# HJakeCunningham/ASVGP

Hardware: NVIDIA B200
Metric: elbo_grad_datapoints_per_s (higher is better)
Workload: dtype f64

## Files before the change

asvgp_b200/csrc/band_engine.cuh:

```cuda
#pragma once
#include "common.cuh"
#include "dual.cuh"

namespace asvgp {

struct ChunkLayout {
    int M, K, P;
    int base, rem;
    ASVGP_HD int size(int p) const { return base + (p < rem ? 1 : 0); }
    ASVGP_HD int start(int p) const { return p * (base + K) + (p < rem ? p : rem); }
    ASVGP_HD int sep_start(int q) const { return start(q) + size(q); }
    ASVGP_HD int max_size() const { return base + (rem > 0 ? 1 : 0); }
    ASVGP_HD int n_reduced() const { return (P - 1) * K; }
};

inline ChunkLayout make_layout(int M, int K, int P) {
    ChunkLayout L;
    L.M = M; L.K = K;
    while (P > 1 && (M - (P - 1) * K) / P < K + 1) --P;
    L.P = P;
    const int interior = M - (P - 1) * K;
    L.base = interior / P;
    L.rem = interior % P;
    return L;
}

inline int default_chunks(int M, int K) {
    if (M < 16 * (K + 1)) return 1;
    int P = M / (4 * (K + 1));
    if (P > 128) P = 128;
    if (P < 1) P = 1;
    return P;
}

template <class T, int K, bool SPIKE = true>
struct ColumnStore {
    T* rec;
    int n_steps, P;
    static constexpr int kFields = SPIKE ? 2 * K + 2 : K + 2;
    static constexpr int kY = kFields - 1;
    ASVGP_HD T& at(int field, int j, int p) const { return rec[((size_t)field * n_steps + j) * P + p]; }
    ASVGP_HD static size_t count(int n_steps, int P) { return (size_t)kFields * n_steps * P; }
};

template <class T, int K>
struct ChunkSchur {
    T logdet, quad;
    T Dend[K][K];
    T rend[K];
    T E[K][K];
    T SLL[K][K];
    T rhsL[K];
    int info;
};

template <class T, int K>
struct WindowRow {
    T a[K + 1];
    T r;
};

template <class T, int K, class MatFn, class RhsFn>
ASVGP_HD void fetch_row(MatFn& A, RhsFn& rhs, int g, WindowRow<T, K>& row) {
#pragma unroll
    for (int b = 0; b <= K; ++b) row.a[b] = A(K - b, g + 1 + b);
    row.r = rhs(g + 1 + K);
}

template <class T, int K, bool SPIKE, bool STORE, class MatFn, class RhsFn, class Store>
ASVGP_HD void eliminate_columns(int g0, int n, int n_steps, MatFn A, RhsFn rhs, const Store& store,
                                int p, ChunkSchur<T, K>& out) {
    T W[K + 1][K + 1];
    T r[K + 1];
    T c[SPIKE ? K : 1][K + 1];
#pragma unroll
    for (int a = 0; a <= K; ++a) {
#pragma unroll
        for (int b = 0; b <= a; ++b) W[a][b] = A(a - b, g0 + b);
        r[a] = rhs(g0 + a);
    }
    if (SPIKE) {
#pragma unroll
        for (int rho = 0; rho < K; ++rho)
#pragma unroll
            for (int a = 0; a <= K; ++a)
                c[rho][a] = (a <= rho) ? A(a + K - rho, g0 - K + rho) : zero_of<T>();
    }
    LogAccum<T> logdet;
    logdet.init();
    T quad = zero_of<T>();
    T SLL[K][K], rhsL[K];
#pragma unroll
    for (int a = 0; a < K; ++a) {
        rhsL[a] = zero_of<T>();
#pragma unroll
        for (int b = 0; b < K; ++b) SLL[a][b] = zero_of<T>();
    }
    int info = 0;

    WindowRow<T, K> rowA, rowB;
    fetch_row<T, K>(A, rhs, g0, rowA);
    fetch_row<T, K>(A, rhs, g0 + 1, rowB);

    auto step = [&](int j, const WindowRow<T, K>& row) {
        const int g = g0 + j;
        if (!(value_of(W[0][0]) > 0.0) && info == 0) info = g + 1;
        const T ip = rsqrt_of(W[0][0]);
        logdet.add(W[0][0], ip);
        T l[K + 1];
#pragma unroll
        for (int a = 1; a <= K; ++a) l[a] = W[a][0] * ip;
        const T yj = r[0] * ip;
        quad += yj * yj;
        T X[SPIKE ? K : 1];
        if (SPIKE) {
#pragma unroll
            for (int rho = 0; rho < K; ++rho) {
                X[rho] = c[rho][0] * ip;
                rhsL[rho] += X[rho] * yj;
#pragma unroll
                for (int r2 = 0; r2 <= rho; ++r2) SLL[rho][r2] += X[rho] * X[r2];
            }
        }
        if (STORE) {
            store.at(0, j, p) = ip;
#pragma unroll
            for (int a = 1; a <= K; ++a) store.at(a, j, p) = l[a];
            if (SPIKE) {
#pragma unroll
                for (int rho = 0; rho < K; ++rho) store.at(K + 1 + rho, j, p) = X[rho];
            }
            store.at(Store::kY, j, p) = yj;
        }
#pragma unroll
        for (int a = 1; a <= K; ++a) {
#pragma unroll
            for (int b = 1; b <= a; ++b) W[a - 1][b - 1] = W[a][b] - l[a] * l[b];
            r[a - 1] = r[a] - l[a] * yj;
            if (SPIKE) {
#pragma unroll
                for (int rho = 0; rho < K; ++rho) c[rho][a - 1] = c[rho][a] - l[a] * X[rho];
            }
        }
#pragma unroll
        for (int b = 0; b <= K; ++b) W[K][b] = row.a[b];
        r[K] = row.r;
        if (SPIKE) {
#pragma unroll
            for (int rho = 0; rho < K; ++rho) c[rho][K] = zero_of<T>();
        }
    };

    for (int j = 0; j < n_steps; j += 2) {
        WindowRow<T, K> nextA, nextB;
        fetch_row<T, K>(A, rhs, g0 + j + 2, nextA);
        if (j < n) step(j, rowA);
        fetch_row<T, K>(A, rhs, g0 + j + 3, nextB);
        if (j + 1 < n) step(j + 1, rowB);
        rowA = nextA;
        rowB = nextB;
    }
    out.logdet = logdet.result();
    out.quad = quad;
    out.info = info;
#pragma unroll
    for (int a = 0; a < K; ++a) {
        out.rend[a] = r[a];
        out.rhsL[a] = rhsL[a];
#pragma unroll
        for (int b = 0; b < K; ++b) {
            out.Dend[a][b] = (b <= a) ? W[a][b] : zero_of<T>();
            out.SLL[a][b] = SLL[a][b];
            out.E[a][b] = SPIKE ? c[b][a] : zero_of<T>();
        }
    }
}

template <class T, int K, class Store>
ASVGP_HD void backsolve_serial(int n, const Store& store, T* x) {
    T xw[K + 1];
#pragma unroll
    for (int a = 0; a <= K; ++a) xw[a] = zero_of<T>();
    for (int j = n - 1; j >= 0; --j) {
        T acc = store.at(Store::kY, j, 0);
#pragma unroll
        for (int a = 1; a <= K; ++a) acc -= store.at(a, j, 0) * xw[a];
        const T xj = acc * store.at(0, j, 0);
#pragma unroll
        for (int a = K; a >= 2; --a) xw[a] = xw[a - 1];
        xw[1] = xj;
        x[j] = xj;
    }
}

template <class T>
struct BandSink {
    T* sig; int M;
    ASVGP_HD void operator()(int d, int col, const T& v) const { sig[(size_t)d * M + col] = v; }
};

template <class T, int K, class Store, class Sink>
ASVGP_HD void selinv_serial(int n, const Store& store, Sink& sink) {
    T Z[K][K];
#pragma unroll
    for (int a = 0; a < K; ++a)
#pragma unroll
        for (int b = 0; b < K; ++b) Z[a][b] = zero_of<T>();
    for (int j = n - 1; j >= 0; --j) {
        const T ip = store.at(0, j, 0);
        T l[K], w[K];
#pragma unroll
        for (int a = 0; a < K; ++a) l[a] = store.at(a + 1, j, 0);
        T dot = zero_of<T>();
#pragma unroll
        for (int a = 0; a < K; ++a) {
            T acc = zero_of<T>();
#pragma unroll
            for (int b = 0; b < K; ++b) acc += Z[a][b] * l[b];
            w[a] = acc;
            dot += l[a] * acc;
        }
        const T ip2 = ip * ip;
        const T sjj = ip2 + dot * ip2;
        sink(0, j, sjj);
        T col[K];
#pragma unroll
        for (int a = 0; a < K; ++a) {
            col[a] = -(w[a] * ip);
            if (j + 1 + a < n) sink(a + 1, j, col[a]);
        }
#pragma unroll
        for (int a = K - 1; a >= 1; --a)
#pragma unroll
            for (int b = K - 1; b >= 1; --b) Z[a][b] = Z[a - 1][b - 1];
        Z[0][0] = sjj;
#pragma unroll
        for (int a = 1; a < K; ++a) { Z[a][0] = col[a - 1]; Z[0][a] = col[a - 1]; }
    }
}

template <class T, int K, bool SOLVE, bool SELINV, class Sink>
ASVGP_HD void chunk_backward(const ChunkLayout& lay, int p, int n_steps, const ColumnStore<T, K, true>& store,
                             const T* x_red, const T* sig_red, T* x_out, Sink& sink) {
    constexpr int KR = 2 * K - 1;
    const int n = lay.size(p), s = lay.start(p), M = lay.M, nred = lay.n_reduced();
    const bool has_left = p > 0, has_right = p < lay.P - 1;
    (void)KR;
    T xw[K + 1], xL[K];
    T Z[2 * K][2 * K];
#pragma unroll
    for (int a = 0; a < K; ++a) {
        xw[a + 1] = (SOLVE && has_right) ? x_red[p * K + a] : zero_of<T>();
        xL[a] = (SOLVE && has_left) ? x_red[(p - 1) * K + a] : zero_of<T>();
    }
    xw[0] = zero_of<T>();
    if (SELINV) {
#pragma unroll
        for (int a = 0; a < 2 * K; ++a)
#pragma unroll
            for (int b = 0; b < 2 * K; ++b) Z[a][b] = zero_of<T>();
#pragma unroll
        for (int a = 0; a < K; ++a) {
#pragma unroll
            for (int b = 0; b <= a; ++b) {
                if (has_right) { Z[a][b] = sig_red[(size_t)(a - b) * nred + p * K + b]; Z[b][a] = Z[a][b]; }
                if (has_left) {
                    Z[K + a][K + b] = sig_red[(size_t)(a - b) * nred + (p - 1) * K + b];
                    Z[K + b][K + a] = Z[K + a][K + b];
                }
            }
#pragma unroll
            for (int rho = 0; rho < K; ++rho) {
                if (has_left && has_right) {
                    Z[a][K + rho] = sig_red[(size_t)(K + a - rho) * nred + (p - 1) * K + rho];
                    Z[K + rho][a] = Z[a][K + rho];
                }
            }
        }
    }
    struct Rec { T ip; T lv[2 * K]; T y; };
    auto fetch = [&](int j, Rec& rec) {
        const int jj = j < 0 ? 0 : (j >= n_steps ? n_steps - 1 : j);
        rec.ip = store.at(0, jj, p);
#pragma unroll
        for (int a = 0; a < K; ++a) {
            rec.lv[a] = store.at(a + 1, jj, p);
            rec.lv[K + a] = store.at(K + 1 + a, jj, p);
        }
        rec.y = store.at(ColumnStore<T, K, true>::kY, jj, p);
    };
    auto step = [&](int j, const Rec& rec) {
        const int g = s + j;
        const T ip = rec.ip;
        if (SOLVE) {
            T acc = rec.y;
#pragma unroll
            for (int a = 0; a < K; ++a) { acc -= rec.lv[a] * xw[a + 1]; acc -= rec.lv[K + a] * xL[a]; }
            const T xj = acc * ip;
#pragma unroll
            for (int a = K; a >= 2; --a) xw[a] = xw[a - 1];
            xw[1] = xj;
            x_out[g] = xj;
        }
        if (SELINV) {
            T w[2 * K];
            T dot = zero_of<T>();
#pragma unroll
            for (int a = 0; a < 2 * K; ++a) {
                T acc = zero_of<T>();
#pragma unroll
                for (int b = 0; b < 2 * K; ++b) acc += Z[a][b] * rec.lv[b];
                w[a] = acc;
                dot += rec.lv[a] * acc;
            }
            const T ip2 = ip * ip;
            const T sjj = ip2 + dot * ip2;
            sink(0, g, sjj);
            T col[2 * K];
#pragma unroll
            for (int a = 0; a < 2 * K; ++a) col[a] = -(w[a] * ip);
#pragma unroll
            for (int a = 0; a < K; ++a) {
                if (g + 1 + a < M) sink(a + 1, g, col[a]);
                if (has_left && j <= a) sink(j + K - a, s - K + a, col[K + a]);
            }
#pragma unroll
            for (int a = K - 1; a >= 1; --a) {
#pragma unroll
                for (int b = K - 1; b >= 1; --b) Z[a][b] = Z[a - 1][b - 1];
#pragma unroll
                for (int rho = 0; rho < K; ++rho) { Z[a][K + rho] = Z[a - 1][K + rho]; Z[K + rho][a] = Z[a][K + rho]; }
            }
            Z[0][0] = sjj;
#pragma unroll
            for (int a = 1; a < K; ++a) { Z[a][0] = col[a - 1]; Z[0][a] = col[a - 1]; }
#pragma unroll
            for (int rho = 0; rho < K; ++rho) { Z[0][K + rho] = col[K + rho]; Z[K + rho][0] = col[K + rho]; }
        }
    };
    Rec recA, recB;
    const int top = ((n_steps + 1) & ~1) - 1;
    fetch(top, recA);
    fetch(top - 1, recB);
    for (int j = top; j >= 0; j -= 2) {
        Rec nextA, nextB;
        fetch(j - 2, nextA);
        if (j < n) step(j, recA);
        fetch(j - 3, nextB);
        if (j - 1 < n && j - 1 >= 0) step(j - 1, recB);
        recA = nextA;
        recB = nextB;
    }
}

}

namespace asvgp {

template <class T, int B>
struct CrNode {
    T D[B][B];
    T E[B][B];
    T Wa[B][B];
    T Wb[B][B];
    T Sa[B][B];
    T Sb[B][B];
    T r[B];
    T ip[B];
    T logdet, quad;
    int info;
};

#if defined(__CUDACC__)
template <class P> __device__ __forceinline__ P* cluster_peer(P* p, int rank) {
    unsigned long long out;
    asm volatile("mapa.u64 %0, %1, %2;" : "=l"(out) : "l"((unsigned long long)p), "r"(rank));
    return reinterpret_cast<P*>(out);
}
#endif

template <class T, int K>
struct ChainWork {
    ColumnStore<T, K, true> cols;
    ChunkSchur<T, K>* schur;
    CrNode<T, K>* nodes;
    T* x_red;
    T* sig_red;
    int per_cta = 0;
    ASVGP_HD ChunkSchur<T, K>& sch(int p) const {
#if defined(__CUDA_ARCH__)
        if (per_cta > 0) return *cluster_peer(schur + p % per_cta, p / per_cta);
#endif
        return schur[p];
    }
    ASVGP_HD CrNode<T, K>& node(int i) const {
#if defined(__CUDA_ARCH__)
        if (per_cta > 0) return *cluster_peer(nodes + i % per_cta, i / per_cta);
#endif
        return nodes[i];
    }
};

template <class T, int K>
struct ChainSmall {
    ASVGP_HD static size_t align16(size_t n) { return (n + 15) & ~(size_t)15; }
    ASVGP_HD static size_t head_bytes(int P) {
        const size_t nred = (size_t)(P - 1) * K + 1;
        const size_t a = align16((size_t)P * sizeof(ChunkSchur<T, K>));
        const size_t b = align16((size_t)(2 * K) * nred * sizeof(T)) + align16(nred * sizeof(T));
        return a > b ? a : b;
    }
    ASVGP_HD static size_t bytes(int P) { return head_bytes(P) + align16((size_t)(P > 1 ? P - 1 : 1) * sizeof(CrNode<T, K>)); }
    ASVGP_HD static void carve(int P, char* base, ChainWork<T, K>& w) {
        const size_t nred = (size_t)(P - 1) * K + 1;
        w.schur = reinterpret_cast<ChunkSchur<T, K>*>(base);
        w.sig_red = reinterpret_cast<T*>(base);
        w.x_red = reinterpret_cast<T*>(base + align16((size_t)(2 * K) * nred * sizeof(T)));
        w.nodes = reinterpret_cast<CrNode<T, K>*>(base + head_bytes(P));
    }
};

template <class T, int K>
struct ChainTotals { T logdet, quad; int info; };

template <class T, int K, bool STORE, class MatFn, class RhsFn>
ASVGP_HD void chain_phase1(const ChunkLayout& lay, int p, MatFn A, RhsFn rhs, const ChainWork<T, K>& w) {
    const int n_steps = lay.max_size();
    if (lay.P == 1) eliminate_columns<T, K, false, STORE>(0, lay.M, n_steps, A, rhs, w.cols, 0, w.sch(0));
    else eliminate_columns<T, K, true, STORE>(lay.start(p), lay.size(p), n_steps, A, rhs, w.cols, p, w.sch(p));
}

template <class T, int K>
ASVGP_HD void cr_assemble(const ChunkLayout& lay, int q, const ChainWork<T, K>& w) {
    const ChunkSchur<T, K>& left = w.sch(q);
    const ChunkSchur<T, K>& right = w.sch(q + 1);
    CrNode<T, K>& nd = w.node(q);
#pragma unroll
    for (int a = 0; a < K; ++a) {
        nd.r[a] = left.rend[a] - right.rhsL[a];
#pragma unroll
        for (int b = 0; b < K; ++b) {
            nd.D[a][b] = (b <= a) ? left.Dend[a][b] - right.SLL[a][b] : zero_of<T>();
            nd.E[a][b] = left.E[a][b];
        }
    }
    nd.logdet = zero_of<T>();
    nd.quad = zero_of<T>();
    nd.info = 0;
}

template <class T, int K>
ASVGP_HD void cr_eliminate(int n, int s, int i, int g_offset, const ChainWork<T, K>& w) {
    CrNode<T, K>& nd = w.node(i);
    const bool has_a = s > 0 && i - s >= 0, has_b = s > 0 && i + s < n;
    T D[K][K], r[K], ipv[K], E[K][K], Eb[K][K];
#pragma unroll
    for (int a = 0; a < K; ++a) {
        r[a] = nd.r[a];
#pragma unroll
        for (int b = 0; b < K; ++b) {
            D[a][b] = (b <= a) ? nd.D[a][b] : zero_of<T>();
            E[a][b] = has_a ? nd.E[a][b] : zero_of<T>();
            Eb[a][b] = has_b ? w.node(i + s).E[a][b] : zero_of<T>();
        }
    }
    LogAccum<T> logdet;
    logdet.init();
    T quad = zero_of<T>();
    int info = 0;
#pragma unroll
    for (int j = 0; j < K; ++j) {
        T d = D[j][j];
#pragma unroll
        for (int q = 0; q < j; ++q) d -= D[j][q] * D[j][q];
        if (!(value_of(d) > 0.0) && info == 0) info = g_offset + i * K + j + 1;
        const T ip = rsqrt_of(d);
        logdet.add(d, ip);
        ipv[j] = ip;
        D[j][j] = d * ip;
#pragma unroll
        for (int rr = j + 1; rr < K; ++rr) {
            T v = D[rr][j];
#pragma unroll
            for (int q = 0; q < j; ++q) v -= D[rr][q] * D[j][q];
            D[rr][j] = v * ip;
        }
        T y = r[j];
#pragma unroll
        for (int q = 0; q < j; ++q) y -= D[j][q] * r[q];
        y = y * ip;
        r[j] = y;
        quad += y * y;
    }
    T Wa[K][K], Wb[K][K];
#pragma unroll
    for (int x = 0; x < K; ++x)
#pragma unroll
        for (int j = 0; j < K; ++j) {
            T va = E[j][x], vb = Eb[x][j];
#pragma unroll
            for (int q = 0; q < j; ++q) { va -= D[j][q] * Wa[x][q]; vb -= D[j][q] * Wb[x][q]; }
            Wa[x][j] = va * ipv[j];
            Wb[x][j] = vb * ipv[j];
        }
#pragma unroll
    for (int a = 0; a < K; ++a) {
        nd.r[a] = r[a];
        nd.ip[a] = ipv[a];
#pragma unroll
        for (int b = 0; b < K; ++b) {
            if (b <= a) nd.D[a][b] = D[a][b];
            if (has_a) nd.Wa[a][b] = Wa[a][b];
            if (has_b) nd.Wb[a][b] = Wb[a][b];
        }
    }
    nd.logdet = logdet.result();
    nd.quad = quad;
    if (info != 0 && nd.info == 0) nd.info = info;
}

template <class T, int K>
ASVGP_HD void cr_update(int n, int s, int c, const ChainWork<T, K>& w) {
    CrNode<T, K>& nd = w.node(c);
    const bool has_p = c + s < n, has_m = c - s >= 0, has_a = c - 2 * s >= 0;
    T D[K][K], r[K], Wp[K][K], yp[K], Wm[K][K], Wma[K][K], ym[K];
#pragma unroll
    for (int a = 0; a < K; ++a) {
        r[a] = nd.r[a];
        yp[a] = has_p ? w.node(c + s).r[a] : zero_of<T>();
        ym[a] = has_m ? w.node(c - s).r[a] : zero_of<T>();
#pragma unroll
        for (int b = 0; b < K; ++b) {
            D[a][b] = (b <= a) ? nd.D[a][b] : zero_of<T>();
            Wp[a][b] = has_p ? w.node(c + s).Wa[a][b] : zero_of<T>();
            Wm[a][b] = has_m ? w.node(c - s).Wb[a][b] : zero_of<T>();
            Wma[a][b] = (has_m && has_a) ? w.node(c - s).Wa[a][b] : zero_of<T>();
        }
    }
#pragma unroll
    for (int x = 0; x < K; ++x) {
        T rr = r[x];
#pragma unroll
        for (int j = 0; j < K; ++j) { rr -= Wp[x][j] * yp[j]; rr -= Wm[x][j] * ym[j]; }
        nd.r[x] = rr;
#pragma unroll
        for (int y = 0; y <= x; ++y) {
            T v = D[x][y];
#pragma unroll
            for (int j = 0; j < K; ++j) { v -= Wp[x][j] * Wp[y][j]; v -= Wm[x][j] * Wm[y][j]; }
            nd.D[x][y] = v;
        }
        if (has_m) {
#pragma unroll
            for (int y = 0; y < K; ++y) {
                T v = zero_of<T>();
#pragma unroll
                for (int j = 0; j < K; ++j) v -= Wm[x][j] * Wma[y][j];
                nd.E[x][y] = v;
            }
        }
    }
}

template <class T, int K, bool SOLVE, bool SELINV>
ASVGP_HD void cr_back(int n, int s, int i, const ChainWork<T, K>& w) {
    CrNode<T, K>& nd = w.node(i);
    const bool has_a = s > 0 && i - s >= 0, has_b = s > 0 && i + s < n;
    const CrNode<T, K>& na = w.node(has_a ? i - s : i);
    const CrNode<T, K>& nb = w.node(has_b ? i + s : i);
    T L[K][K], ipv[K], Wa[K][K], Wb[K][K];
#pragma unroll
    for (int a = 0; a < K; ++a) {
        ipv[a] = nd.ip[a];
#pragma unroll
        for (int b = 0; b < K; ++b) {
            L[a][b] = (b <= a) ? nd.D[a][b] : zero_of<T>();
            Wa[a][b] = has_a ? nd.Wa[a][b] : zero_of<T>();
            Wb[a][b] = has_b ? nd.Wb[a][b] : zero_of<T>();
        }
    }
    if (SOLVE) {
        T t[K], xa[K], xb[K];
#pragma unroll
        for (int j = 0; j < K; ++j) {
            t[j] = nd.r[j];
            xa[j] = has_a ? na.r[j] : zero_of<T>();
            xb[j] = has_b ? nb.r[j] : zero_of<T>();
        }
#pragma unroll
        for (int j = 0; j < K; ++j) {
            T v = t[j];
#pragma unroll
            for (int x = 0; x < K; ++x) { v -= Wa[x][j] * xa[x]; v -= Wb[x][j] * xb[x]; }
            t[j] = v;
        }
#pragma unroll
        for (int j = K - 1; j >= 0; --j) {
            T v = t[j];
#pragma unroll
            for (int q = j + 1; q < K; ++q) v -= L[q][j] * t[q];
            t[j] = v * ipv[j];
        }
#pragma unroll
        for (int j = 0; j < K; ++j) nd.r[j] = t[j];
    }
    if (SELINV) {
        const bool both = has_a && has_b;
        const bool a_is_odd = both && (((i - s) / (2 * s)) & 1);
        T Saa[K][K], Sbb[K][K], Sba[K][K];
#pragma unroll
        for (int x = 0; x < K; ++x)
#pragma unroll
            for (int y = 0; y < K; ++y) {
                Saa[x][y] = has_a ? na.D[x][y] : zero_of<T>();
                Sbb[x][y] = has_b ? nb.D[x][y] : zero_of<T>();
                Sba[x][y] = both ? (a_is_odd ? na.Sb[x][y] : nb.Sa[y][x]) : zero_of<T>();
            }
        T Li[K][K];
#pragma unroll
        for (int c = 0; c < K; ++c)
#pragma unroll
            for (int r = 0; r < K; ++r) {
                if (r < c) { Li[r][c] = zero_of<T>(); continue; }
                T v = (r == c) ? make_scalar<T>(1.0, 0.0) : zero_of<T>();
#pragma unroll
                for (int q = c; q < r; ++q) v -= L[r][q] * Li[q][c];
                Li[r][c] = v * ipv[r];
            }
        T Ya[K][K], Yb[K][K];
#pragma unroll
        for (int x = 0; x < K; ++x)
#pragma unroll
            for (int c = 0; c < K; ++c) {
                T va = zero_of<T>(), vb = zero_of<T>();
#pragma unroll
                for (int j = c; j < K; ++j) { va += Wa[x][j] * Li[j][c]; vb += Wb[x][j] * Li[j][c]; }
                Ya[x][c] = va;
                Yb[x][c] = vb;
            }
        T Sai[K][K], Sbi[K][K];
#pragma unroll
        for (int x = 0; x < K; ++x)
#pragma unroll
            for (int c = 0; c < K; ++c) {
                T va = zero_of<T>(), vb = zero_of<T>();
#pragma unroll
                for (int y = 0; y < K; ++y) {
                    va -= Saa[x][y] * Ya[y][c];
                    va -= Sba[y][x] * Yb[y][c];
                    vb -= Sba[x][y] * Ya[y][c];
                    vb -= Sbb[x][y] * Yb[y][c];
                }
                Sai[x][c] = va;
                Sbi[x][c] = vb;
            }
#pragma unroll
        for (int c = 0; c < K; ++c)
#pragma unroll
            for (int c2 = 0; c2 < K; ++c2) {
                T v = zero_of<T>();
#pragma unroll
                for (int r = 0; r < K; ++r) {
                    if (r >= c && r >= c2) v += Li[r][c] * Li[r][c2];
                }
#pragma unroll
                for (int x = 0; x < K; ++x) { v -= Ya[x][c] * Sai[x][c2]; v -= Yb[x][c] * Sbi[x][c2]; }
                nd.D[c][c2] = v;
                if (has_a) nd.Sa[c][c2] = Sai[c][c2];
                if (has_b) nd.Sb[c][c2] = Sbi[c][c2];
            }
    }
}

template <class T, int K, bool SOLVE, bool SELINV>
ASVGP_HD void cr_export(const ChunkLayout& lay, int q, const ChainWork<T, K>& w) {
    const int nred = lay.n_reduced();
    const CrNode<T, K>& nd = w.node(q);
    if (SOLVE) {
#pragma unroll
        for (int a = 0; a < K; ++a) w.x_red[q * K + a] = nd.r[a];
    }
    if (SELINV) {
#pragma unroll
        for (int a = 0; a < K; ++a)
#pragma unroll
            for (int b = 0; b <= a; ++b) w.sig_red[(size_t)(a - b) * nred + q * K + b] = nd.D[a][b];
        if (q >= 1) {
            const bool q_odd = q & 1;
            const CrNode<T, K>& prev = w.node(q - 1);
#pragma unroll
            for (int a = 0; a < K; ++a)
#pragma unroll
                for (int rho = 0; rho < K; ++rho)
                    w.sig_red[(size_t)(K + a - rho) * nred + (q - 1) * K + rho] = q_odd ? nd.Sa[rho][a] : prev.Sb[a][rho];
        }
    }
}

template <class T, int K>
ASVGP_HD ChainTotals<T, K> chain_totals(const ChunkLayout& lay, const ChainWork<T, K>& w) {
    ChainTotals<T, K> tot;
    tot.logdet = zero_of<T>();
    tot.quad = zero_of<T>();
    tot.info = 0;
    for (int p = 0; p < lay.P; ++p) {
        tot.logdet += w.sch(p).logdet;
        tot.quad += w.sch(p).quad;
        if (w.sch(p).info != 0 && (tot.info == 0 || w.sch(p).info < tot.info)) tot.info = w.sch(p).info;
    }
    for (int q = 0; q + 1 < lay.P; ++q) {
        tot.logdet += w.node(q).logdet;
        tot.quad += w.node(q).quad;
        if (w.node(q).info != 0 && tot.info == 0) tot.info = w.node(q).info;
    }
    return tot;
}

ASVGP_HD int cr_top_stride(int n) {
    int s = 1;
    while (2 * s < n) s *= 2;
    return n > 1 ? s : 0;
}

template <class T, int K, bool SOLVE, bool SELINV, class Sink>
ASVGP_HD void chain_phase3(const ChunkLayout& lay, int p, const ChainWork<T, K>& w, T* x_out, Sink& sink) {
    const int n_steps = lay.max_size();
    if (lay.P == 1) {
        if (SOLVE) backsolve_serial<T, K>(lay.M, w.cols, x_out);
        if (SELINV) selinv_serial<T, K>(lay.M, w.cols, sink);
        return;
    }
    const int nred = lay.n_reduced();
    if (p < lay.P - 1) {
        const int g = lay.sep_start(p);
        for (int a = 0; a < K; ++a) {
            if (SOLVE) x_out[g + a] = w.x_red[p * K + a];
            if (SELINV)
                for (int b = 0; b <= a; ++b)
                    sink(a - b, g + b, w.sig_red[(size_t)(a - b) * nred + p * K + b]);
        }
    }
    chunk_backward<T, K, SOLVE, SELINV>(lay, p, n_steps, w.cols, w.x_red, w.sig_red, x_out, sink);
}

}
```

asvgp_b200/csrc/banded_1d.cu:

```cuda
#include <cooperative_groups.h>
#include <cuda_runtime.h>

#include <cstdio>
#include <cstdlib>

#include <algorithm>

#include "band_engine.cuh"
#include "../../include/asvgp_b200.h"

namespace asvgp {

constexpr int kChainThreads = 128;

__device__ __forceinline__ void pdl_wait() { asm volatile("griddepcontrol.wait;" ::: "memory"); }
__device__ __forceinline__ void pdl_launch_dependents() { asm volatile("griddepcontrol.launch_dependents;" ::: "memory"); }
constexpr int kMaxTerms = 12;

struct KuuTerms {
    int n_terms;
    double coef[kMaxTerms];
    double dcoef[kMaxTerms];
};

__global__ void __launch_bounds__(256) kuu_assemble_kernel(const double* __restrict__ tables, KuuTerms terms,
                                                           int64_t band_elems, double* __restrict__ Kuu,
                                                           double* __restrict__ dKuu) {
    for (int64_t i = blockIdx.x * (int64_t)blockDim.x + threadIdx.x; i < band_elems;
         i += (int64_t)gridDim.x * blockDim.x) {
        double v = 0.0, dv = 0.0;
        for (int t = 0; t < terms.n_terms; ++t) {
            const double s = __ldg(tables + (int64_t)t * band_elems + i);
            v = __dadd_rn(v, __dmul_rn(terms.coef[t], s));
            dv = __dadd_rn(dv, __dmul_rn(terms.dcoef[t], s));
        }
        Kuu[i] = v;
        if (dKuu != nullptr) dKuu[i] = dv;
    }
}

template <class T> struct BandMat;
template <> struct BandMat<Dual<1>> {
    const double* Kuu; const double* dKuu; const double* G;
    double beta, tb; int use_dK; int M;
    __device__ __forceinline__ Dual<1> operator()(int d, int j) const {
        const bool ok = (j >= 0) & (j + d < M);
        const size_t i = ok ? (size_t)d * M + j : 0;
        const double kv = __ldg(Kuu + i);
        const double dk = use_dK ? __ldg(dKuu + i) : 0.0;
        const double g = (G != nullptr) ? __ldg(G + i) : 0.0;
        Dual<1> r;
        r.v = ok ? fma(beta, g, kv) : 0.0;
        r.d[0] = ok ? fma(tb, g, dk) : 0.0;
        return r;
    }
};
template <> struct BandMat<double> {
    const double* Kuu; const double* dKuu; const double* G;
    double beta, tb; int use_dK; int M;
    __device__ __forceinline__ double operator()(int d, int j) const {
        const bool ok = (j >= 0) & (j + d < M);
        const size_t i = ok ? (size_t)d * M + j : 0;
        const double kv = __ldg(Kuu + i);
        const double g = (G != nullptr) ? __ldg(G + i) : 0.0;
        return ok ? fma(beta, g, kv) : 0.0;
    }
};
template <class T> struct VecRhs {
    const double* b; int M; int use;
    __device__ __forceinline__ T operator()(int j) const {
        const bool ok = (use != 0) & (j >= 0) & (j < M);
        const double v = __ldg(b + (ok ? j : 0));
        return make_scalar<T>(ok ? v : 0.0, 0.0);
    }
};

template <class T, int K>
struct RowsMat {
    const T* rows; int g0, P, p, n_rho;
    __device__ __forceinline__ T operator()(int d, int col) const {
        const int rho = col + d - g0;
        const bool ok = (rho >= 0) & (rho < n_rho);
        const T v = rows[ok ? ((size_t)rho * (K + 1) + (K - d)) * P + p : (size_t)p];
        return ok ? v : zero_of<T>();
    }
};
template <class T>
struct RowsRhs {
    const T* r; int g0, P, p, n_rho;
    __device__ __forceinline__ T operator()(int j) const {
        const int rho = j - g0;
        const bool ok = (rho >= 0) & (rho < n_rho);
        const T v = r[ok ? (size_t)rho * P + p : (size_t)p];
        return ok ? v : zero_of<T>();
    }
};
__host__ __device__ inline int chain_n_rho(const ChunkLayout& lay, int K) { return lay.max_size() + K + 4; }
template <class T, int K>
__host__ __device__ inline size_t chain_rows_count(const ChunkLayout& lay) {
    return (size_t)chain_n_rho(lay, K) * (K + 2) * lay.P;
}

template <class T> struct ChainSpec { BandMat<T> A; VecRhs<T> rhs; };

constexpr int kTraceBlocks = 64, kTraceThreads = 256, kTraceUnroll = 4;
struct TraceJob {
    const double* kstate;
    const double* G;
    double* tr_part;
    int M, K, first_block;
};
__device__ __forceinline__ void trace_partial(const double* __restrict__ kstate, const double* __restrict__ G, int M, int K, int block,
                                              double* __restrict__ tr_part) {
    __shared__ double s_tr[2][kTraceThreads / 32];
    const Dual<1>* kinv = reinterpret_cast<const Dual<1>*>(kstate + 16);
    double tr = 0.0, dtr_dl = 0.0;
    const int band = (K + 1) * M, stride = kTraceThreads * kTraceBlocks;
    for (int i0 = block * kTraceThreads + threadIdx.x; i0 < band; i0 += stride * kTraceUnroll) {
        Dual<1> sv[kTraceUnroll];
        double gv[kTraceUnroll];
#pragma unroll
        for (int u = 0; u < kTraceUnroll; ++u) {
            const int i = i0 + u * stride;
            const int d = i / M, col = i - d * M;
            const bool ok = i < band && col + d < M;
            sv[u] = kinv[ok ? i : 0];
            gv[u] = ok ? (d == 0 ? 1.0 : 2.0) * G[i] : 0.0;
        }
#pragma unroll
        for (int u = 0; u < kTraceUnroll; ++u) {
            if (gv[u] != 0.0) { tr = fma(sv[u].v, gv[u], tr); dtr_dl = fma(sv[u].d[0], gv[u], dtr_dl); }
        }
    }
#pragma unroll
    for (int o = 16; o > 0; o >>= 1) {
        tr += __shfl_xor_sync(0xffffffffu, tr, o);
        dtr_dl += __shfl_xor_sync(0xffffffffu, dtr_dl, o);
    }
    if ((threadIdx.x & 31) == 0) { s_tr[0][threadIdx.x >> 5] = tr; s_tr[1][threadIdx.x >> 5] = dtr_dl; }
    __syncthreads();
    if (threadIdx.x == 0) {
        tr = 0.0; dtr_dl = 0.0;
        for (int i = 0; i < kTraceThreads / 32; ++i) { tr += s_tr[0][i]; dtr_dl += s_tr[1][i]; }
        tr_part[2 * block] = tr; tr_part[2 * block + 1] = dtr_dl;
    }
}

template <class T, int K, int NCHAINS>
__global__ void __launch_bounds__(256) chain_rows_kernel(ChunkLayout lay, ChainSpec<T> s0, ChainSpec<T> s1, ChainSpec<T> s2, ChainSpec<T> s3,
                                                         T* __restrict__ out, unsigned* __restrict__ zero_me = nullptr,
                                                         TraceJob trace = TraceJob{nullptr, nullptr, nullptr, 0, 0, 0}) {
    pdl_launch_dependents();
    if (zero_me != nullptr && blockIdx.x == 0 && threadIdx.x == 0) *zero_me = 0u;
    if (trace.kstate != nullptr && (int)blockIdx.x >= trace.first_block) {
        trace_partial(trace.kstate, trace.G, trace.M, trace.K, (int)blockIdx.x - trace.first_block, trace.tr_part);
        return;
    }
    const unsigned n_rho = chain_n_rho(lay, K), P = lay.P;
    const unsigned per_chain = (unsigned)chain_rows_count<T, K>(lay);
    const unsigned total = per_chain * NCHAINS;
    const unsigned n_row_blocks = trace.kstate != nullptr ? (unsigned)trace.first_block : gridDim.x;
    for (unsigned t = blockIdx.x * blockDim.x + threadIdx.x; t < total; t += n_row_blocks * blockDim.x) {
        const unsigned chain = t / per_chain;
        const unsigned e = t - chain * per_chain;
        const ChainSpec<T>& sp = chain == 0 ? s0 : (chain == 1 ? s1 : (chain == 2 ? s2 : s3));
        const unsigned q = e / P;
        const int p = (int)(e - q * P);
        const int g0 = P > 1 ? lay.start(p) : 0;
        if (q < n_rho * (K + 1)) {
            const int rho = (int)(q / (K + 1)), bidx = (int)(q - (unsigned)rho * (K + 1));
            const int row = g0 + rho, col = row - K + bidx;
            out[t] = sp.A(K - bidx, col);
        } else {
            const int rho = (int)(q - n_rho * (K + 1));
            out[t] = sp.rhs(g0 + rho);
        }
    }
}

template <class T, int K>
struct ChainPlan {
    static size_t bytes(const ChunkLayout& lay) {
        const size_t n = ColumnStore<T, K, true>::count(lay.max_size(), lay.P) * sizeof(T);
        return (n + 255) & ~(size_t)255;
    }
    static ColumnStore<T, K, true> carve(const ChunkLayout& lay, char* base) {
        return ColumnStore<T, K, true>{reinterpret_cast<T*>(base), lay.max_size(), lay.P};
    }
};

constexpr size_t kChainSmemLimit = 200 * 1024;

template <class T, int K, bool STORE, bool SOLVE, bool SELINV, class Mat, class Rhs, class Sink>
__device__ __forceinline__ void run_chain(const ChunkLayout& lay, const ColumnStore<T, K, true>& cols, char* smem,
                                          Mat A, Rhs rhs, T* x_out, Sink& sink, ChainTotals<T, K>* tot,
                                          long long* clk) {
    const int p = threadIdx.x;
    ChainWork<T, K> w;
    w.cols = cols;
    ChainSmall<T, K>::carve(lay.P, smem, w);
    if (p == 0 && clk) clk[0] = clock64();
    if (p < lay.P) chain_phase1<T, K, STORE>(lay, p, A, rhs, w);
    __syncthreads();
    if (p == 0 && clk) clk[1] = clock64();
    const int n = lay.P - 1;
    if (p < n) cr_assemble<T, K>(lay, p, w);
    __syncthreads();
    for (int s = 1; s < n; s *= 2) {
        if (p < n && (p & (2 * s - 1)) == s) cr_eliminate<T, K>(n, s, p, lay.M, w);
        __syncthreads();
        if (p < n && (p & (2 * s - 1)) == 0) cr_update<T, K>(n, s, p, w);
        __syncthreads();
    }
    if (p == 0) {
        if (n > 0) cr_eliminate<T, K>(n, 0, 0, lay.M, w);
        *tot = chain_totals<T, K>(lay, w);
        if ((SOLVE || SELINV) && n > 0) cr_back<T, K, SOLVE, SELINV>(n, 0, 0, w);
    }
    __syncthreads();
    if ((SOLVE || SELINV) && n > 0) {
        for (int s = cr_top_stride(n); s >= 1; s /= 2) {
            if (p < n && (p & (2 * s - 1)) == s) cr_back<T, K, SOLVE, SELINV>(n, s, p, w);
            __syncthreads();
        }
        if (p < n) cr_export<T, K, SOLVE, SELINV>(lay, p, w);
        __syncthreads();
    }
    if (p == 0 && clk) clk[2] = clock64();
    if ((SOLVE || SELINV) && p < lay.P) chain_phase3<T, K, SOLVE, SELINV>(lay, p, w, x_out, sink);
    __syncthreads();
    if (p == 0 && clk) clk[3] = clock64();
}

template <class T, int K, bool STORE, bool SOLVE, bool SELINV, class MakeMat, class MakeRhs, class MakeSink>
__device__ __forceinline__ void run_chain_cluster(const ChunkLayout& lay, const ColumnStore<T, K, true>& cols, char* smem, T* red_scratch,
                                                  MakeMat make_A, MakeRhs make_rhs, MakeSink make_sink, T* x_out,
                                                  ChainTotals<T, K>* tot, long long* clk) {
    namespace cg = cooperative_groups;
    cg::cluster_group cluster = cg::this_cluster();
    const int rank = (int)cluster.block_rank(), n_cta = (int)cluster.num_blocks();
    const int tid = threadIdx.x;
    const int per = kChainThreads;
    const int p = rank * per + tid;
    ChainWork<T, K> w;
    w.cols = cols;
    ChainSmall<T, K>::carve(per + 1, smem, w);
    w.per_cta = per;
    const size_t nred = (size_t)lay.n_reduced();
    w.sig_red = red_scratch;
    w.x_red = red_scratch + (size_t)(2 * K) * nred;
#ifdef ASVGP_CHAIN_TRACE
    __shared__ long long s_trace[64];
    int n_trace = 0;
#define ASVGP_STAMP() do { if (rank == 0 && tid == 0 && n_trace < 64) s_trace[n_trace++] = clock64(); } while (0)
#else
#define ASVGP_STAMP() do {} while (0)
#endif
    cluster.sync();
    ASVGP_STAMP();
    if (rank == 0 && tid == 0 && clk) clk[0] = clock64();
    if (p < lay.P) chain_phase1<T, K, STORE>(lay, p, make_A(p), make_rhs(p), w);
    cluster.sync();
    ASVGP_STAMP();
    if (rank == 0 && tid == 0 && clk) clk[1] = clock64();
    const int n = lay.P - 1;
    if (p < n) cr_assemble<T, K>(lay, p, w);
    cluster.sync();
    ASVGP_STAMP();
    for (int s = 1; s < n; s *= 2) {
        if (p < n && (p & (2 * s - 1)) == s) cr_eliminate<T, K>(n, s, p, lay.M, w);
        cluster.sync();
        ASVGP_STAMP();
        if (p < n && (p & (2 * s - 1)) == 0) cr_update<T, K>(n, s, p, w);
        cluster.sync();
        ASVGP_STAMP();
    }
    if (p == 0 && n > 0) cr_eliminate<T, K>(n, 0, 0, lay.M, w);
    cluster.sync();
    ASVGP_STAMP();
    {
        T ld = zero_of<T>(), qd = zero_of<T>();
        int info = 0;
        if (p < lay.P) { const ChunkSchur<T, K>& c = w.sch(p); ld += c.logdet; qd += c.quad; info = c.info; }
        if (p < n) { const CrNode<T, K>& nd = w.node(p); ld += nd.logdet; qd += nd.quad; if (info == 0) info = nd.info; }
        double v[4] = {value_of(ld), tangent_of(ld, 0), value_of(qd), tangent_of(qd, 0)};
        unsigned uinfo = info == 0 ? 0xffffffffu : (unsigned)info;
#pragma unroll
        for (int o = 16; o > 0; o >>= 1) {
#pragma unroll
            for (int i = 0; i < 4; ++i) v[i] += __shfl_xor_sync(0xffffffffu, v[i], o);
            uinfo = min(uinfo, __shfl_xor_sync(0xffffffffu, uinfo, o));
        }
        __shared__ double s_tot[kChainThreads / 32][4];
        __shared__ unsigned s_info[kChainThreads / 32];
        __shared__ double s_cta[5];
        if ((tid & 31) == 0) { for (int i = 0; i < 4; ++i) s_tot[tid >> 5][i] = v[i]; s_info[tid >> 5] = uinfo; }
        __syncthreads();
        if (tid == 0) {
            double a[4] = {0, 0, 0, 0};
            unsigned ui = 0xffffffffu;
            for (int wv = 0; wv < kChainThreads / 32; ++wv) { for (int i = 0; i < 4; ++i) a[i] += s_tot[wv][i]; ui = min(ui, s_info[wv]); }
            for (int i = 0; i < 4; ++i) s_cta[i] = a[i];
            s_cta[4] = (double)ui;
        }
        cluster.sync();
        ASVGP_STAMP();
        if (rank == 0 && tid == 0) {
            double a[4] = {0, 0, 0, 0};
            double ui = 4294967295.0;
            for (int r = 0; r < n_cta; ++r) {
                const double* q = cluster_peer(s_cta, r);
                for (int i = 0; i < 4; ++i) a[i] += q[i];
                ui = q[4] < ui ? q[4] : ui;
            }
            tot->logdet = make_scalar<T>(a[0], a[1]);
            tot->quad = make_scalar<T>(a[2], a[3]);
            tot->info = ui >= 4294967295.0 ? 0 : (int)ui;
        }
    }
    if ((SOLVE || SELINV) && n > 0) {
        if (p == 0) cr_back<T, K, SOLVE, SELINV>(n, 0, 0, w);
        cluster.sync();
        ASVGP_STAMP();
        for (int s = cr_top_stride(n); s >= 1; s /= 2) {
            if (p < n && (p & (2 * s - 1)) == s) cr_back<T, K, SOLVE, SELINV>(n, s, p, w);
            cluster.sync();
            ASVGP_STAMP();
        }
        if (p < n) cr_export<T, K, SOLVE, SELINV>(lay, p, w);
        __threadfence();
        cluster.sync();
        ASVGP_STAMP();
    }
    if (rank == 0 && tid == 0 && clk) clk[2] = clock64();
    if ((SOLVE || SELINV) && p < lay.P) {
        auto sink = make_sink(p);
        chain_phase3<T, K, SOLVE, SELINV>(lay, p, w, x_out, sink);
    }
    cluster.sync();
    ASVGP_STAMP();
    if (rank == 0 && tid == 0 && clk) clk[3] = clock64();
#ifdef ASVGP_CHAIN_TRACE
    if (rank == 0 && tid == 0) {
        for (int i = 1; i < n_trace; ++i) printf("trace blk=%d SELINV=%d P=%d step=%d %lld\n", (int)blockIdx.x, (int)SELINV, lay.P, i, s_trace[i] - s_trace[i - 1]);
    }
#endif
#undef ASVGP_STAMP
}

template <int K>
struct ElboArgs {
    ChunkLayout lay;
    int first_chain;
    ColumnStore<Dual<1>, K, true> cols[2];
    double* partial[2];
    const Dual<1>* rows;
    Dual<1>* kinv;
};

template <int K>
__global__ void __launch_bounds__(kChainThreads) elbo_chains_kernel(ElboArgs<K> a) {
    using T = Dual<1>;
    extern __shared__ __align__(16) char smem[];
    const int slot = blockIdx.x, chain = a.first_chain + slot, p = threadIdx.x;
    const ChunkLayout lay = a.lay;
    const int M = lay.M;
    __shared__ ChainTotals<T, K> tot;
    __shared__ long long clk[4];
    double* out = a.partial[slot];
    pdl_launch_dependents();
    pdl_wait();

    const int n_rho = chain_n_rho(lay, K), g0 = lay.P > 1 ? lay.start(p < lay.P ? p : 0) : 0, pp = p < lay.P ? p : 0;
    const T* tab = a.rows + (size_t)slot * chain_rows_count<T, K>(lay);
    const RowsMat<T, K> A{tab, g0, lay.P, pp, n_rho};
    const RowsRhs<T> rhs{tab + (size_t)n_rho * (K + 1) * lay.P, g0, lay.P, pp, n_rho};
    if (chain == 0) {
        BandSink<T> sink{a.kinv, M};
        run_chain<T, K, true, false, true>(lay, a.cols[slot], smem, A, rhs, static_cast<T*>(nullptr), sink, &tot, clk);
    } else {
        BandSink<T> no_sink{nullptr, M};
        run_chain<T, K, false, false, false>(lay, a.cols[slot], smem, A, rhs, static_cast<T*>(nullptr), no_sink, &tot, clk);
    }
    if (p == 0) {
        out[0] = tot.logdet.v; out[1] = tot.logdet.d[0];
        out[2] = tot.quad.v;   out[3] = tot.quad.d[0];
        out[6] = (double)tot.info;
        const long long t_end = clock64();
        out[8] = (double)(clk[1] - clk[0]); out[9] = (double)(clk[2] - clk[1]);
        out[10] = (double)(clk[3] - clk[2]); out[11] = (double)(t_end - clk[3]);
    }
}

template <int K, int NCTA>
__global__ void __cluster_dims__(NCTA, 1, 1) __launch_bounds__(kChainThreads) elbo_chains_cluster_kernel(ElboArgs<K> a, Dual<1>* red_scratch) {
    using T = Dual<1>;
    extern __shared__ __align__(16) char smem[];
    const int slot = blockIdx.x / NCTA, chain = a.first_chain + slot, rank = blockIdx.x % NCTA, tid = threadIdx.x;
    const ChunkLayout lay = a.lay;
    __shared__ ChainTotals<T, K> tot;
    __shared__ long long clk[4];
    double* out = a.partial[slot];
    pdl_launch_dependents();
    pdl_wait();
    const int n_rho = chain_n_rho(lay, K);
    const T* tab = a.rows + (size_t)slot * chain_rows_count<T, K>(lay);
    T* scratch = red_scratch + (size_t)slot * ((size_t)(2 * K + 1) * lay.n_reduced() + 8);
    auto g0_of = [&](int lane) { return lay.P > 1 ? lay.start(lane) : 0; };
    auto make_A = [&](int lane) { return RowsMat<T, K>{tab, g0_of(lane), lay.P, lane, n_rho}; };
    auto make_rhs = [&](int lane) { return RowsRhs<T>{tab + (size_t)n_rho * (K + 1) * lay.P, g0_of(lane), lay.P, lane, n_rho}; };
    if (chain == 0) {
        auto make_sink = [&](int) { return BandSink<T>{a.kinv, lay.M}; };
        run_chain_cluster<T, K, true, false, true>(lay, a.cols[slot], smem, scratch, make_A, make_rhs, make_sink, static_cast<T*>(nullptr), &tot, clk);
    } else {
        auto make_sink = [&](int) { return BandSink<T>{nullptr, lay.M}; };
        run_chain_cluster<T, K, false, false, false>(lay, a.cols[slot], smem, scratch, make_A, make_rhs, make_sink, static_cast<T*>(nullptr), &tot, clk);
    }
    if (rank == 0 && tid == 0) {
        out[0] = tot.logdet.v; out[1] = tot.logdet.d[0];
        out[2] = tot.quad.v;   out[3] = tot.quad.d[0];
        out[6] = (double)tot.info;
        const long long t_end = clock64();
        out[8] = (double)(clk[1] - clk[0]); out[9] = (double)(clk[2] - clk[1]);
        out[10] = (double)(clk[3] - clk[2]); out[11] = (double)(t_end - clk[3]);
    }
}

__global__ void __launch_bounds__(kTraceThreads) elbo_finalize_kernel(const double* __restrict__ kstate, double* __restrict__ partial,
                                                                      const double* __restrict__ G, const double* __restrict__ scal,
                                                                      int M, int K, double variance, double sigma2, int trace_done,
                                                                      double* __restrict__ out) {
    double* tr_part = partial + 64;
    unsigned* counter = reinterpret_cast<unsigned*>(partial + 32);
    pdl_wait();
    if (!trace_done) {
        trace_partial(kstate, G, M, K, (int)blockIdx.x, tr_part);
        if (threadIdx.x != 0) return;
        __threadfence();
        if (atomicAdd(counter, 1u) != gridDim.x - 1) return;
        __threadfence();
    } else if (threadIdx.x != 0) {
        return;
    }
    double tr = 0.0, dtr_dl = 0.0;
    for (int i = 0; i < kTraceBlocks; ++i) { tr += __ldcg(tr_part + 2 * i); dtr_dl += __ldcg(tr_part + 2 * i + 1); }
    const double* cK = kstate;
    const double* cL = partial;
    const double* cS = partial + 16;
    const double yy = scal[0], N = scal[1];
    const double v = variance, s2 = sigma2;
    const double logdetK = cK[0], dlogdetK_dl = cK[1];
    const double logdetP = cL[0], dlogdetP_dl = cL[1], Q = cL[2], dQ_dl = cL[3];
    const double dlogdetP_ds = cS[1], dQ_ds = cS[3];
    const double two_pi = 6.283185307179586476925286766559;
    const double elbo = -0.5 * N * log(two_pi * s2) - 0.5 * logdetP + 0.5 * logdetK - 0.5 * yy / s2
                        + 0.5 * Q / (s2 * s2) - 0.5 * N * v / s2 + 0.5 * tr / s2;
    const double d_l = -0.5 * dlogdetP_dl + 0.5 * dlogdetK_dl + 0.5 * dQ_dl / (s2 * s2) + 0.5 * dtr_dl / s2;
    const double d_s = -0.5 * N / s2 - 0.5 * dlogdetP_ds + 0.5 * yy / (s2 * s2) + 0.5 * dQ_ds / (s2 * s2)
                       - Q / (s2 * s2 * s2) + 0.5 * N * v / (s2 * s2) - 0.5 * tr / (s2 * s2);
    const double dlogdetP_dv = -(double)M / v - (s2 / v) * dlogdetP_ds;
    const double dQ_dv = Q / v - (s2 / v) * dQ_ds;
    const double d_v = -0.5 * dlogdetP_dv - 0.5 * (double)M / v + 0.5 * dQ_dv / (s2 * s2) - 0.5 * N / s2
                       + 0.5 * tr / (v * s2);
    out[0] = elbo; out[1] = d_v; out[2] = d_l; out[3] = d_s;
    out[4] = logdetK; out[5] = logdetP; out[6] = Q; out[7] = tr;
    double info = cK[6];
    if (info == 0.0) info = cL[6];
    if (info == 0.0) info = cS[6];
    out[8] = info;
    out[9] = cK[8]; out[10] = cK[9]; out[11] = cK[10]; out[12] = cK[11];
    out[13] = cL[8]; out[14] = cL[9];
    out[15] = dtr_dl;
}

template <int K>
struct PosteriorArgs {
    ChunkLayout lay;
    ColumnStore<double, K, true> cols[2];
    const double* Kuu; const double* G; const double* b;
    double sigma2;
    double* sigK; double* sigP; double* x;
    double* info;
    const double* rows;
};

template <int K>
__global__ void __launch_bounds__(kChainThreads) posterior_chains_kernel(PosteriorArgs<K> a) {
    using T = double;
    extern __shared__ __align__(16) char smem[];
    const int chain = blockIdx.x, p = threadIdx.x;
    const ChunkLayout lay = a.lay;
    const int M = lay.M;
    __shared__ ChainTotals<T, K> tot;
    (void)M;
    const int n_rho = chain_n_rho(lay, K), g0 = lay.P > 1 ? lay.start(p < lay.P ? p : 0) : 0, pp = p < lay.P ? p : 0;
    const T* tab = a.rows + (size_t)chain * chain_rows_count<T, K>(lay);
    const RowsMat<T, K> A{tab, g0, lay.P, pp, n_rho};
    const RowsRhs<T> rhs{tab + (size_t)n_rho * (K + 1) * lay.P, g0, lay.P, pp, n_rho};
    BandSink<T> sinkK{a.sigK, lay.M}, sinkP{a.sigP, lay.M};
    if (chain == 0) run_chain<T, K, true, false, true>(lay, a.cols[0], smem, A, rhs, static_cast<T*>(nullptr), sinkK, &tot, nullptr);
    else run_chain<T, K, true, true, true>(lay, a.cols[1], smem, A, rhs, a.x, sinkP, &tot, nullptr);
    if (p == 0) a.info[chain] = (double)tot.info;
}

__global__ void __launch_bounds__(256) posterior_combine_kernel(const double* __restrict__ sigK,
                                                                const double* __restrict__ sigP,
                                                                const double* __restrict__ x, double inv_s2, int M,
                                                                int band_elems, double* __restrict__ alpha,
                                                                double* __restrict__ S) {
    for (int i = blockIdx.x * blockDim.x + threadIdx.x; i < band_elems; i += gridDim.x * blockDim.x) {
        S[i] = sigP[i] - sigK[i];
        if (i < M) alpha[i] = x[i] * inv_s2;
    }
}


template <int K>
struct BandInvArgs {
    ChunkLayout lay;
    ColumnStore<Dual<1>, K, true> cols;
    const double* A; const double* dA;
    Dual<1>* sig;
    double* sig_val; double* sig_tan;
    double* scal;
    const Dual<1>* rows;
};

template <int K>
__global__ void __launch_bounds__(kChainThreads) band_inverse_kernel(BandInvArgs<K> a) {
    using T = Dual<1>;
    extern __shared__ __align__(16) char smem[];
    const int p = threadIdx.x;
    const ChunkLayout lay = a.lay;
    const int M = lay.M;
    __shared__ ChainTotals<T, K> tot;
    const int n_rho = chain_n_rho(lay, K), g0 = lay.P > 1 ? lay.start(p < lay.P ? p : 0) : 0, pp = p < lay.P ? p : 0;
    const RowsMat<T, K> A{a.rows, g0, lay.P, pp, n_rho};
    const RowsRhs<T> rhs{a.rows + (size_t)n_rho * (K + 1) * lay.P, g0, lay.P, pp, n_rho};
    BandSink<T> sink{a.sig, lay.M};
    run_chain<T, K, true, false, true>(lay, a.cols, smem, A, rhs, static_cast<T*>(nullptr), sink, &tot, nullptr);
    for (int i = p; i < (K + 1) * M; i += kChainThreads) {
        const T s = a.sig[i];
        a.sig_val[i] = s.v;
        a.sig_tan[i] = s.d[0];
    }
    if (p == 0) {
        a.scal[0] = tot.logdet.v; a.scal[1] = tot.logdet.d[0]; a.scal[2] = (double)tot.info; a.scal[3] = 0.0;
    }
}

template <int K>
static int launch_band_inverse(const ChunkLayout& lay, const double* A, const double* dA, double* sig_val,
                               double* sig_tan, double* scal, char* work, cudaStream_t st) {
    BandInvArgs<K> a;
    a.lay = lay;
    char* p = work;
    a.cols = ChainPlan<Dual<1>, K>::carve(lay, p);
    p += ChainPlan<Dual<1>, K>::bytes(lay);
    a.sig = reinterpret_cast<Dual<1>*>(p);
    a.A = A; a.dA = dA; a.sig_val = sig_val; a.sig_tan = sig_tan; a.scal = scal;
    p += ((size_t)(K + 1) * lay.M * sizeof(Dual<1>) + 255) & ~(size_t)255;
    Dual<1>* rows = reinterpret_cast<Dual<1>*>(p);
    a.rows = rows;
    {
        using T = Dual<1>;
        ChainSpec<T> s0{BandMat<T>{A, dA, nullptr, 0.0, 0.0, 1, lay.M}, VecRhs<T>{A, lay.M, 0}};
        const size_t total = chain_rows_count<T, K>(lay);
        chain_rows_kernel<T, K, 1><<<(int)((total + 255) / 256), 256, 0, st>>>(lay, s0, s0, s0, s0, rows); ASVGP_LAUNCHED();
        ASVGP_CUDA_OK(cudaGetLastError());
    }
    ASVGP_CUDA_OK(cudaMemsetAsync(a.sig, 0, (size_t)(K + 1) * lay.M * sizeof(Dual<1>), st));
    const size_t smem = ChainSmall<Dual<1>, K>::bytes(lay.P);
    ASVGP_CUDA_OK(cudaFuncSetAttribute(band_inverse_kernel<K>, cudaFuncAttributeMaxDynamicSharedMemorySize, (int)smem));
    band_inverse_kernel<K><<<1, kChainThreads, smem, st>>>(a); ASVGP_LAUNCHED();
    ASVGP_CUDA_OK(cudaGetLastError());
    return kOk;
}

static size_t align256(size_t n) { return (n + 255) & ~(size_t)255; }
template <class... KArgs, class... Args>
static cudaError_t launch_dependent(void (*kernel)(KArgs...), int grid, int block, size_t smem, cudaStream_t st, bool pdl, Args... args) {
    cudaLaunchConfig_t cfg = {};
    cfg.gridDim = dim3(grid); cfg.blockDim = dim3(block); cfg.dynamicSmemBytes = smem; cfg.stream = st;
    cudaLaunchAttribute attr[1];
    attr[0].id = cudaLaunchAttributeProgrammaticStreamSerialization;
    attr[0].val.programmaticStreamSerializationAllowed = 1;
    cfg.attrs = attr; cfg.numAttrs = pdl ? 1 : 0;
    return cudaLaunchKernelEx(&cfg, kernel, KArgs(args)...);
}
template <class Kernel>
static cudaError_t allow_smem(Kernel kernel, size_t smem) {
    static size_t allowed = 0;
    static const void* which = nullptr;
    if (which == reinterpret_cast<const void*>(kernel) && smem <= allowed) return cudaSuccess;
    const cudaError_t e = cudaFuncSetAttribute(kernel, cudaFuncAttributeMaxDynamicSharedMemorySize, (int)smem);
    if (e == cudaSuccess) { allowed = smem; which = reinterpret_cast<const void*>(kernel); }
    return e;
}
constexpr size_t kPartialBytes = 2048;
template <int K>
static size_t red_scratch_count(const ChunkLayout& lay) { return (size_t)(2 * K + 1) * lay.n_reduced() + 8; }
template <int K>
static size_t chains_work_bytes(const ChunkLayout& lay, int n_chains) {
    return n_chains * ChainPlan<Dual<1>, K>::bytes(lay) + kPartialBytes + align256(n_chains * chain_rows_count<Dual<1>, K>(lay) * sizeof(Dual<1>))
           + align256(n_chains * red_scratch_count<K>(lay) * sizeof(Dual<1>));
}
static size_t kuu_state_doubles(int M, int K) { return 16 + 2 * (size_t)(K + 1) * M; }
template <int K>
static size_t elbo_work_bytes(const ChunkLayout& lay) {
    return chains_work_bytes<K>(lay, 1) + chains_work_bytes<K>(lay, 2) + align256(kuu_state_doubles(lay.M, K) * sizeof(double));
}
template <int K>
static size_t posterior_work_bytes(const ChunkLayout& lay) {
    return 2 * ChainPlan<double, K>::bytes(lay) + 3 * ((((size_t)(K + 1) * lay.M * sizeof(double)) + 255) & ~(size_t)255)
           + 256 + (((size_t)lay.M * sizeof(double) + 255) & ~(size_t)255) + 2 * chain_rows_count<double, K>(lay) * sizeof(double) + 256;
}

template <int K>
static int launch_chain_group(const ChunkLayout& lay, int first_chain, int n_chains, const ChainSpec<Dual<1>>& s0,
                              const ChainSpec<Dual<1>>& s1, double* partial0, Dual<1>* kinv, char* work, double** partials_out,
                              cudaEvent_t gate, TraceJob trace, cudaStream_t st) {
    using T = Dual<1>;
    ElboArgs<K> a;
    a.lay = lay;
    a.first_chain = first_chain;
    a.kinv = kinv;
    char* p = work;
    for (int c = 0; c < 2; ++c) {
        a.cols[c] = ChainPlan<T, K>::carve(lay, c < n_chains ? p : work);
        if (c < n_chains) p += ChainPlan<T, K>::bytes(lay);
    }
    double* partial = reinterpret_cast<double*>(p);
    p += kPartialBytes;
    a.partial[0] = partial0 != nullptr ? partial0 : partial;
    a.partial[1] = partial + 16;
    if (partials_out != nullptr) *partials_out = partial;
    T* rows = reinterpret_cast<T*>(p);
    p += align256(n_chains * chain_rows_count<T, K>(lay) * sizeof(T));
    a.rows = rows;
    T* scratch = reinterpret_cast<T*>(p);
    const size_t total = n_chains * chain_rows_count<T, K>(lay);
    ASVGP_REQUIRE(total < ((size_t)1 << 31), "banded chains: %zu row-table entries exceed the 32-bit index range", total);
    const int grid = (int)std::min<size_t>((total + 255) / 256, 148 * 8);
    if (n_chains == 1) {
        chain_rows_kernel<T, K, 1><<<grid, 256, 0, st>>>(lay, s0, s0, s0, s0, rows);
    } else {
        trace.first_block = grid;
        trace.tr_part = partial + 64;
        chain_rows_kernel<T, K, 2><<<grid + (trace.kstate != nullptr ? kTraceBlocks : 0), 256, 0, st>>>(
            lay, s0, s1, s1, s1, rows, reinterpret_cast<unsigned*>(partial + 32), trace);
    }
    ASVGP_LAUNCHED();
    ASVGP_CUDA_OK(cudaGetLastError());
    if (gate != nullptr) ASVGP_CUDA_OK(cudaEventRecord(gate, st));
    const int n_cta = (lay.P + kChainThreads - 1) / kChainThreads;
    const bool pdl = gate == nullptr;
    const size_t smem_floor = gate != nullptr ? (size_t)(227 * 1024 - 2048) : 0;
    if (n_cta > 1) {
        const size_t smem = std::max(ChainSmall<T, K>::bytes(kChainThreads + 1), smem_floor);
        if (n_cta == 2) {
            ASVGP_CUDA_OK(allow_smem(elbo_chains_cluster_kernel<K, 2>, smem));
            ASVGP_CUDA_OK(launch_dependent(elbo_chains_cluster_kernel<K, 2>, n_chains * 2, kChainThreads, smem, st, pdl, a, scratch));
        } else if (n_cta == 8) {
            ASVGP_CUDA_OK(allow_smem(elbo_chains_cluster_kernel<K, 8>, smem));
            ASVGP_CUDA_OK(launch_dependent(elbo_chains_cluster_kernel<K, 8>, n_chains * 8, kChainThreads, smem, st, pdl, a, scratch));
        } else {
            ASVGP_CUDA_OK(allow_smem(elbo_chains_cluster_kernel<K, 4>, smem));
            ASVGP_CUDA_OK(launch_dependent(elbo_chains_cluster_kernel<K, 4>, n_chains * 4, kChainThreads, smem, st, pdl, a, scratch));
        }
    } else {
        const size_t smem = std::max(ChainSmall<T, K>::bytes(lay.P), smem_floor);
        ASVGP_CUDA_OK(allow_smem(elbo_chains_kernel<K>, smem));
        ASVGP_CUDA_OK(launch_dependent(elbo_chains_kernel<K>, n_chains, kChainThreads, smem, st, pdl, a));
    }
    ASVGP_LAUNCHED();
    ASVGP_CUDA_OK(cudaGetLastError());
    return kOk;
}

template <int K>
static int launch_kuu_chain(const ChunkLayout& lay, const double* Kuu, const double* dKuu, double* kstate, char* work, cudaEvent_t gate,
                            cudaStream_t st) {
    using T = Dual<1>;
    const int M = lay.M;
    ChainSpec<T> s0{BandMat<T>{Kuu, dKuu, nullptr, 0.0, 0.0, 1, M}, VecRhs<T>{Kuu, M, 0}};
    return launch_chain_group<K>(lay, 0, 1, s0, s0, kstate, reinterpret_cast<T*>(kstate + 16), work, nullptr, gate,
                                 TraceJob{nullptr, nullptr, nullptr, 0, 0, 0}, st);
}

template <int K>
static int launch_pchains(const ChunkLayout& lay, const double* kstate, const double* Kuu, const double* dKuu, const double* acc,
                          double variance, double sigma2, double* out, char* work, cudaEvent_t kuu_ready, int join_late, cudaStream_t st) {
    using T = Dual<1>;
    const int M = lay.M;
    const double* G = acc;
    const double* b = acc + (size_t)(K + 1) * M;
    const double inv_s2 = 1.0 / sigma2;
    ChainSpec<T> s1{BandMat<T>{Kuu, dKuu, G, inv_s2, 0.0, 1, M}, VecRhs<T>{b, M, 1}};
    ChainSpec<T> s2{BandMat<T>{Kuu, dKuu, G, inv_s2, -inv_s2 * inv_s2, 0, M}, VecRhs<T>{b, M, 1}};
    double* partial = nullptr;
    if (!join_late && kuu_ready != nullptr) ASVGP_CUDA_OK(cudaStreamWaitEvent(st, kuu_ready, 0));
    const TraceJob trace{join_late ? nullptr : kstate, G, nullptr, M, K, 0};
    if (int rc = launch_chain_group<K>(lay, 1, 2, s1, s2, nullptr, nullptr, work, &partial, nullptr, trace, st)) return rc;
    if (join_late && kuu_ready != nullptr) ASVGP_CUDA_OK(cudaStreamWaitEvent(st, kuu_ready, 0));
    const bool pdl = !(join_late && kuu_ready != nullptr);
    ASVGP_CUDA_OK(launch_dependent(elbo_finalize_kernel, join_late ? kTraceBlocks : 1, kTraceThreads, 0, st, pdl, kstate, partial, G,
                                   acc + (size_t)(K + 2) * M, M, K, variance, sigma2, join_late ? 0 : 1, out));
    ASVGP_LAUNCHED();
    ASVGP_CUDA_OK(cudaGetLastError());
    return kOk;
}

template <int K>
static int launch_elbo(const ChunkLayout& lay, const double* Kuu, const double* dKuu, const double* acc,
                       double variance, double sigma2, double* out, char* work, cudaStream_t st) {
    double* kstate = reinterpret_cast<double*>(work + chains_work_bytes<K>(lay, 1));
    char* pwork = work + chains_work_bytes<K>(lay, 1) + align256(kuu_state_doubles(lay.M, K) * sizeof(double));
    if (int rc = launch_kuu_chain<K>(lay, Kuu, dKuu, kstate, work, nullptr, st)) return rc;
    return launch_pchains<K>(lay, kstate, Kuu, dKuu, acc, variance, sigma2, out, pwork, nullptr, 0, st);
}

template <int K>
static int launch_posterior(const ChunkLayout& lay, const double* Kuu, const double* acc, double sigma2,
                            double* alpha, double* S, double* info, char* work, cudaStream_t st) {
    PosteriorArgs<K> a;
    a.lay = lay;
    char* p = work;
    for (int c = 0; c < 2; ++c) { a.cols[c] = ChainPlan<double, K>::carve(lay, p); p += ChainPlan<double, K>::bytes(lay); }
    const int M = lay.M;
    const size_t band_bytes = (((size_t)(K + 1) * M * sizeof(double)) + 255) & ~(size_t)255;
    a.sigK = reinterpret_cast<double*>(p); p += band_bytes;
    a.sigP = reinterpret_cast<double*>(p); p += band_bytes;
    a.x = reinterpret_cast<double*>(p);
    p += ((size_t)M * sizeof(double) + 255) & ~(size_t)255;
    a.Kuu = Kuu; a.G = acc; a.b = acc + (size_t)(K + 1) * M;
    a.sigma2 = sigma2;
    a.info = info;
    {
        using T = double;
        T* rows = reinterpret_cast<T*>(p);
        a.rows = rows;
        ChainSpec<T> s0{BandMat<T>{Kuu, nullptr, nullptr, 0.0, 0.0, 0, M}, VecRhs<T>{Kuu, M, 0}};
        ChainSpec<T> s1{BandMat<T>{Kuu, nullptr, a.G, 1.0 / sigma2, 0.0, 0, M}, VecRhs<T>{a.b, M, 1}};
        const size_t total = 2 * chain_rows_count<T, K>(lay);
        chain_rows_kernel<T, K, 2><<<(int)std::min<size_t>((total + 255) / 256, 148 * 8), 256, 0, st>>>(lay, s0, s1, s1, s1, rows); ASVGP_LAUNCHED();
        ASVGP_CUDA_OK(cudaGetLastError());
    }
    ASVGP_CUDA_OK(cudaMemsetAsync(a.sigK, 0, 2 * band_bytes, st));
    const size_t smem = ChainSmall<double, K>::bytes(lay.P);
    ASVGP_CUDA_OK(cudaFuncSetAttribute(posterior_chains_kernel<K>, cudaFuncAttributeMaxDynamicSharedMemorySize, (int)smem));
    posterior_chains_kernel<K><<<2, kChainThreads, smem, st>>>(a); ASVGP_LAUNCHED();
    ASVGP_CUDA_OK(cudaGetLastError());
    const int band_elems = (K + 1) * M;
    posterior_combine_kernel<<<(band_elems + 255) / 256, 256, 0, st>>>(a.sigK, a.sigP, a.x, 1.0 / sigma2, M, band_elems,
                                                                      alpha, S); ASVGP_LAUNCHED();
    ASVGP_CUDA_OK(cudaGetLastError());
    return kOk;
}

template <int K>
static int max_chunks_for_smem() {
    int P = kChainThreads;
    while (P > 1 && ChainSmall<Dual<1>, K>::bytes(P) > kChainSmemLimit) --P;
    return P;
}

static ChunkLayout pick_layout(int M, int K, int chunks) {
    int P = chunks > 0 ? chunks : default_chunks(M, K);
    int cap = kChainThreads;
    switch (K) {
        case 1: cap = max_chunks_for_smem<1>(); break;
        case 2: cap = max_chunks_for_smem<2>(); break;
        case 3: cap = max_chunks_for_smem<3>(); break;
        case 4: cap = max_chunks_for_smem<4>(); break;
        case 5: cap = max_chunks_for_smem<5>(); break;
        case 6: cap = max_chunks_for_smem<6>(); break;
    }
    if (P > cap) P = cap;
    return make_layout(M, K, P);
}

static ChunkLayout pick_layout_elbo(int M, int K, int chunks) {
    const bool explicit_cluster = chunks == 2 * kChainThreads || chunks == 4 * kChainThreads || chunks == 8 * kChainThreads;
    const ChunkLayout one = pick_layout(M, K, explicit_cluster ? 0 : chunks);
    if ((chunks != 0 && !explicit_cluster) || one.P < kChainThreads) return one;
    int n_cta = explicit_cluster ? chunks / kChainThreads : 8;
    if (const char* e = getenv("ASVGP_CHAIN_CTAS")) n_cta = atoi(e);
    if (n_cta != 2 && n_cta != 4 && n_cta != 8) return one;
    int P = M / (2 * (K + 1) + 1);
    while (n_cta > 1 && P < kChainThreads * n_cta) n_cta /= 2;
    if (n_cta <= 1) return one;
    return make_layout(M, K, kChainThreads * n_cta);
}

}

using namespace asvgp;

#define ASVGP_DISPATCH_ORDER(order, CALL)                         \
    switch (order) {                                              \
        case 1: { constexpr int K = 1; CALL; } break;             \
        case 2: { constexpr int K = 2; CALL; } break;             \
        case 3: { constexpr int K = 3; CALL; } break;             \
        case 4: { constexpr int K = 4; CALL; } break;             \
        case 5: { constexpr int K = 5; CALL; } break;             \
        case 6: { constexpr int K = 6; CALL; } break;             \
        default:                                                  \
            set_last_error("spline order %d not in 1..6", order); \
            return kBadArgument;                                  \
    }

extern "C" int asvgp_kuu_assemble(const double* tables, int n_terms, const double* h_coef, const double* h_dcoef,
                                  int M, int order, double* Kuu, double* dKuu, void* stream) {
    ASVGP_REQUIRE(n_terms >= 1 && n_terms <= kMaxTerms, "kuu_assemble: n_terms=%d not in 1..%d", n_terms, kMaxTerms);
    ASVGP_REQUIRE(M > 0 && order >= 1 && order <= kMaxOrder, "kuu_assemble: M=%d order=%d", M, order);
    KuuTerms t;
    t.n_terms = n_terms;
    for (int i = 0; i < n_terms; ++i) { t.coef[i] = h_coef[i]; t.dcoef[i] = h_dcoef ? h_dcoef[i] : 0.0; }
    const int64_t elems = (int64_t)(order + 1) * M;
    const int blocks = (int)((elems + 255) / 256);
    kuu_assemble_kernel<<<blocks, 256, 0, static_cast<cudaStream_t>(stream)>>>(tables, t, elems, Kuu, dKuu); ASVGP_LAUNCHED();
    ASVGP_CUDA_OK(cudaGetLastError());
    return kOk;
}

extern "C" int64_t asvgp_workspace_bytes_1d(int M, int order, int chunks) {
    if (M <= 0 || order < 1 || order > kMaxOrder) return -1;
    const ChunkLayout lay = pick_layout(M, order, chunks > kChainThreads ? 0 : chunks);
    ChunkLayout cand[4] = {lay, lay, lay, lay};
    int n_cand = 1;
    if ((chunks == 0 || chunks == 2 * kChainThreads || chunks == 4 * kChainThreads || chunks == 8 * kChainThreads) && lay.P >= kChainThreads) {
        const int P = M / (2 * (order + 1) + 1);
        if (P >= 2 * kChainThreads) cand[n_cand++] = make_layout(M, order, 2 * kChainThreads);
        if (P >= 4 * kChainThreads) cand[n_cand++] = make_layout(M, order, 4 * kChainThreads);
        if (P >= 8 * kChainThreads) cand[n_cand++] = make_layout(M, order, 8 * kChainThreads);
    }
    size_t e = 0, p = 0;
    for (int c = 0; c < n_cand; ++c) {
        size_t ec = 0;
        switch (order) {
            case 1: ec = elbo_work_bytes<1>(cand[c]); p = posterior_work_bytes<1>(lay); break;
            case 2: ec = elbo_work_bytes<2>(cand[c]); p = posterior_work_bytes<2>(lay); break;
            case 3: ec = elbo_work_bytes<3>(cand[c]); p = posterior_work_bytes<3>(lay); break;
            case 4: ec = elbo_work_bytes<4>(cand[c]); p = posterior_work_bytes<4>(lay); break;
            case 5: ec = elbo_work_bytes<5>(cand[c]); p = posterior_work_bytes<5>(lay); break;
            case 6: ec = elbo_work_bytes<6>(cand[c]); p = posterior_work_bytes<6>(lay); break;
        }
        e = ec > e ? ec : e;
    }
    return (int64_t)(e > p ? e : p);
}

extern "C" int asvgp_elbo_grad_1d(const double* Kuu, const double* dKuu, const double* acc, int M, int order,
                                  double variance, double sigma2, int chunks, double* out, void* work,
                                  int64_t work_bytes, void* stream) {
    ASVGP_REQUIRE(M > 2 * order && order >= 1 && order <= kMaxOrder, "elbo_grad_1d: M=%d order=%d", M, order);
    ASVGP_REQUIRE(variance > 0.0 && sigma2 > 0.0, "elbo_grad_1d: variance=%g sigma2=%g must be positive", variance, sigma2);
    ASVGP_REQUIRE(work_bytes >= asvgp_workspace_bytes_1d(M, order, chunks), "elbo_grad_1d: workspace too small");
    const ChunkLayout lay = pick_layout_elbo(M, order, chunks);
    cudaStream_t st = static_cast<cudaStream_t>(stream);
    ASVGP_DISPATCH_ORDER(order, { if (int rc = launch_elbo<K>(lay, Kuu, dKuu, acc, variance, sigma2, out,
                                                              static_cast<char*>(work), st)) return rc; });
    return kOk;
}

extern "C" int64_t asvgp_kuu_state_doubles(int M, int order) {
    if (M <= 0 || order < 1 || order > kMaxOrder) return -1;
    return (int64_t)kuu_state_doubles(M, order);
}

extern "C" int asvgp_kuu_chain_1d(const double* Kuu, const double* dKuu, int M, int order, int chunks, double* kuu_state,
                                  void* work, int64_t work_bytes, void* gate_event, void* stream) {
    ASVGP_REQUIRE(M > 2 * order && order >= 1 && order <= kMaxOrder, "kuu_chain_1d: M=%d order=%d", M, order);
    ASVGP_REQUIRE(work_bytes >= asvgp_workspace_bytes_1d(M, order, chunks), "kuu_chain_1d: workspace too small");
    const ChunkLayout lay = pick_layout_elbo(M, order, chunks);
    cudaStream_t st = static_cast<cudaStream_t>(stream);
    ASVGP_DISPATCH_ORDER(order, { if (int rc = launch_kuu_chain<K>(lay, Kuu, dKuu, kuu_state, static_cast<char*>(work),
                                                                   static_cast<cudaEvent_t>(gate_event), st)) return rc; });
    return kOk;
}

extern "C" int asvgp_elbo_grad_1d_prepared(const double* kuu_state, const double* Kuu, const double* dKuu, const double* acc,
                                           int M, int order, double variance, double sigma2, int chunks, double* out,
                                           void* work, int64_t work_bytes, void* kuu_ready_event, int join_late, void* stream) {
    ASVGP_REQUIRE(M > 2 * order && order >= 1 && order <= kMaxOrder, "elbo_grad_1d_prepared: M=%d order=%d", M, order);
    ASVGP_REQUIRE(variance > 0.0 && sigma2 > 0.0, "elbo_grad_1d_prepared: variance=%g sigma2=%g must be positive", variance, sigma2);
    ASVGP_REQUIRE(work_bytes >= asvgp_workspace_bytes_1d(M, order, chunks), "elbo_grad_1d_prepared: workspace too small");
    const ChunkLayout lay = pick_layout_elbo(M, order, chunks);
    cudaStream_t st = static_cast<cudaStream_t>(stream);
    ASVGP_DISPATCH_ORDER(order, { if (int rc = launch_pchains<K>(lay, kuu_state, Kuu, dKuu, acc, variance, sigma2, out, static_cast<char*>(work),
                                                                 static_cast<cudaEvent_t>(kuu_ready_event), join_late, st)) return rc; });
    return kOk;
}

extern "C" int asvgp_posterior_1d(const double* Kuu, const double* acc, int M, int order, double sigma2, int chunks,
                                  double* alpha, double* S_band, double* info, void* work, int64_t work_bytes,
                                  void* stream) {
    ASVGP_REQUIRE(M > 2 * order && order >= 1 && order <= kMaxOrder, "posterior_1d: M=%d order=%d", M, order);
    ASVGP_REQUIRE(sigma2 > 0.0, "posterior_1d: sigma2=%g must be positive", sigma2);
    ASVGP_REQUIRE(work_bytes >= asvgp_workspace_bytes_1d(M, order, chunks), "posterior_1d: workspace too small");
    const ChunkLayout lay = pick_layout(M, order, chunks);
    cudaStream_t st = static_cast<cudaStream_t>(stream);
    ASVGP_DISPATCH_ORDER(order, { if (int rc = launch_posterior<K>(lay, Kuu, acc, sigma2, alpha, S_band, info,
                                                                   static_cast<char*>(work), st)) return rc; });
    return kOk;
}

extern "C" int asvgp_band_inverse_1d(const double* A, const double* dA, int M, int order, int chunks, double* sig_val,
                                     double* sig_tan, double* scal, void* work, int64_t work_bytes, void* stream) {
    ASVGP_REQUIRE(M > 2 * order && order >= 1 && order <= kMaxOrder, "band_inverse_1d: M=%d order=%d", M, order);
    ASVGP_REQUIRE(work_bytes >= asvgp_workspace_bytes_1d(M, order, chunks), "band_inverse_1d: workspace too small");
    const ChunkLayout lay = pick_layout(M, order, chunks);
    cudaStream_t st = static_cast<cudaStream_t>(stream);
    ASVGP_DISPATCH_ORDER(order, { if (int rc = launch_band_inverse<K>(lay, A, dA, sig_val, sig_tan, scal,
                                                                      static_cast<char*>(work), st)) return rc; });
    return kOk;
}
```

Measured before the change: 290.9 billion.

## Fuse ELBO chain row-building, trace and finalize into single pchains kernel

Splits the Kuu chain into its own kernel and replaces the rows-table kernel, chain kernels and finalize kernel for the posterior chains with one fused pchains kernel. That kernel computes the trace with extra CTAs and uses an arrival ticket so the last arriver finalizes. Cyclic-reduction elimination and update are factored into node-level helpers, and grouped CR helpers are added for a hierarchical reduction. The aim is fewer launches and no round trip through a global row table, at the cost of more complex synchronisation and larger kernels.

```diff
diff --git a/asvgp_b200/csrc/band_engine.cuh b/asvgp_b200/csrc/band_engine.cuh
--- a/asvgp_b200/csrc/band_engine.cuh
+++ b/asvgp_b200/csrc/band_engine.cuh
@@ -450,9 +450,8 @@
 }
 
 template <class T, int K>
-ASVGP_HD void cr_eliminate(int n, int s, int i, int g_offset, const ChainWork<T, K>& w) {
-    CrNode<T, K>& nd = w.node(i);
-    const bool has_a = s > 0 && i - s >= 0, has_b = s > 0 && i + s < n;
+ASVGP_HD void cr_eliminate_node(CrNode<T, K>& nd, const CrNode<T, K>* nb, bool has_a, int info_base) {
+    const bool has_b = nb != nullptr;
     T D[K][K], r[K], ipv[K], E[K][K], Eb[K][K];
 #pragma unroll
     for (int a = 0; a < K; ++a) {
@@ -461,7 +460,7 @@
         for (int b = 0; b < K; ++b) {
             D[a][b] = (b <= a) ? nd.D[a][b] : zero_of<T>();
             E[a][b] = has_a ? nd.E[a][b] : zero_of<T>();
-            Eb[a][b] = has_b ? w.node(i + s).E[a][b] : zero_of<T>();
+            Eb[a][b] = has_b ? nb->E[a][b] : zero_of<T>();
         }
     }
     LogAccum<T> logdet;
@@ -473,7 +472,7 @@
         T d = D[j][j];
 #pragma unroll
         for (int q = 0; q < j; ++q) d -= D[j][q] * D[j][q];
-        if (!(value_of(d) > 0.0) && info == 0) info = g_offset + i * K + j + 1;
+        if (!(value_of(d) > 0.0) && info == 0) info = info_base + j + 1;
         const T ip = rsqrt_of(d);
         logdet.add(d, ip);
         ipv[j] = ip;
@@ -520,21 +519,26 @@
 }
 
 template <class T, int K>
-ASVGP_HD void cr_update(int n, int s, int c, const ChainWork<T, K>& w) {
-    CrNode<T, K>& nd = w.node(c);
-    const bool has_p = c + s < n, has_m = c - s >= 0, has_a = c - 2 * s >= 0;
+ASVGP_HD void cr_eliminate(int n, int s, int i, int g_offset, const ChainWork<T, K>& w) {
+    const bool has_a = s > 0 && i - s >= 0, has_b = s > 0 && i + s < n;
+    cr_eliminate_node<T, K>(w.node(i), has_b ? &w.node(i + s) : nullptr, has_a, g_offset + i * K);
+}
+
+template <class T, int K>
+ASVGP_HD void cr_update_node(CrNode<T, K>& nd, const CrNode<T, K>* np, const CrNode<T, K>* nm, bool has_a) {
+    const bool has_p = np != nullptr, has_m = nm != nullptr;
     T D[K][K], r[K], Wp[K][K], yp[K], Wm[K][K], Wma[K][K], ym[K];
 #pragma unroll
     for (int a = 0; a < K; ++a) {
         r[a] = nd.r[a];
-        yp[a] = has_p ? w.node(c + s).r[a] : zero_of<T>();
-        ym[a] = has_m ? w.node(c - s).r[a] : zero_of<T>();
+        yp[a] = has_p ? np->r[a] : zero_of<T>();
+        ym[a] = has_m ? nm->r[a] : zero_of<T>();
 #pragma unroll
         for (int b = 0; b < K; ++b) {
             D[a][b] = (b <= a) ? nd.D[a][b] : zero_of<T>();
-            Wp[a][b] = has_p ? w.node(c + s).Wa[a][b] : zero_of<T>();
-            Wm[a][b] = has_m ? w.node(c - s).Wb[a][b] : zero_of<T>();
-            Wma[a][b] = (has_m && has_a) ? w.node(c - s).Wa[a][b] : zero_of<T>();
+            Wp[a][b] = has_p ? np->Wa[a][b] : zero_of<T>();
+            Wm[a][b] = has_m ? nm->Wb[a][b] : zero_of<T>();
+            Wma[a][b] = (has_m && has_a) ? nm->Wa[a][b] : zero_of<T>();
         }
     }
 #pragma unroll
@@ -560,6 +564,12 @@
             }
         }
     }
+}
+
+template <class T, int K>
+ASVGP_HD void cr_update(int n, int s, int c, const ChainWork<T, K>& w) {
+    const bool has_p = c + s < n, has_m = c - s >= 0, has_a = c - 2 * s >= 0;
+    cr_update_node<T, K>(w.node(c), has_p ? &w.node(c + s) : nullptr, has_m ? &w.node(c - s) : nullptr, has_a);
 }
 
 template <class T, int K, bool SOLVE, bool SELINV>
@@ -722,6 +732,72 @@
     return n > 1 ? s : 0;
 }
 
+struct CrGroup {
+    int n, gs, r;
+    ASVGP_HD static int count(int n, int gs) { return n / gs + 1; }
+    ASVGP_HD int lo() const { return r > 0 ? 0 : 1; }
+    ASVGP_HD int hi() const { const int h = n - gs * r; return h < gs ? h : gs; }
+    ASVGP_HD int node(int j) const { return gs * r + j - 1; }
+    ASVGP_HD bool eliminates(int s, int j) const { return j >= 1 && j < gs && j <= hi() && (j & (2 * s - 1)) == s; }
+    ASVGP_HD bool updates(int s, int c) const { return c >= lo() && c <= hi() && (c & (2 * s - 1)) == 0; }
+};
+
+template <class T, int K>
+ASVGP_HD void crg_assemble(const CrGroup& g, int j, const ChunkSchur<T, K>* sch, CrNode<T, K>* loc) {
+    const ChunkSchur<T, K>* left = j > 0 ? &sch[j - 1] : nullptr;
+    const ChunkSchur<T, K>* right = j < g.gs ? &sch[j] : nullptr;
+    CrNode<T, K>& nd = loc[j];
+#pragma unroll
+    for (int a = 0; a < K; ++a) {
+        nd.r[a] = (left ? left->rend[a] : zero_of<T>()) - (right ? right->rhsL[a] : zero_of<T>());
+#pragma unroll
+        for (int b = 0; b < K; ++b) {
+            nd.D[a][b] = (b <= a) ? (left ? left->Dend[a][b] : zero_of<T>()) - (right ? right->SLL[a][b] : zero_of<T>()) : zero_of<T>();
+            nd.E[a][b] = left ? left->E[a][b] : zero_of<T>();
+        }
+    }
+    nd.logdet = zero_of<T>();
+    nd.quad = zero_of<T>();
+    nd.info = 0;
+}
+
+template <class T, int K>
+ASVGP_HD void crg_eliminate(const CrGroup& g, int s, int j, int g_offset, CrNode<T, K>* loc) {
+    cr_eliminate_node<T, K>(loc[j], j + s <= g.hi() ? &loc[j + s] : nullptr, j - s >= g.lo(), g_offset + g.node(j) * K);
+}
+
+template <class T, int K>
+ASVGP_HD void crg_update(const CrGroup& g, int s, int c, CrNode<T, K>* loc) {
+    cr_update_node<T, K>(loc[c], c + s <= g.hi() ? &loc[c + s] : nullptr, c - s >= g.lo() ? &loc[c - s] : nullptr, c - 2 * s >= g.lo());
+}
+
+template <class T, int K>
+ASVGP_HD void crg_top_assemble(int t, const CrNode<T, K>& end, const CrNode<T, K>& begin, CrNode<T, K>& top) {
+#pragma unroll
+    for (int a = 0; a < K; ++a) {
+        top.r[a] = end.r[a] + begin.r[a];
+#pragma unroll
+        for (int b = 0; b < K; ++b) {
+            top.D[a][b] = (b <= a) ? end.D[a][b] + begin.D[a][b] : zero_of<T>();
+            top.E[a][b] = t > 0 ? end.E[a][b] : zero_of<T>();
+        }
+    }
+    top.logdet = zero_of<T>();
+    top.quad = zero_of<T>();
+    top.info = 0;
+}
+
+template <class T, int K>
+ASVGP_HD void crg_top_eliminate(int nt, int s, int t, int gs, int g_offset, CrNode<T, K>* top) {
+    const bool has_a = s > 0 && t - s >= 0, has_b = s > 0 && t + s < nt;
+    cr_eliminate_node<T, K>(top[t], has_b ? &top[t + s] : nullptr, has_a, g_offset + (gs * t + gs - 1) * K);
+}
+
+template <class T, int K>
+ASVGP_HD void crg_top_update(int nt, int s, int c, CrNode<T, K>* top) {
+    cr_update_node<T, K>(top[c], c + s < nt ? &top[c + s] : nullptr, c - s >= 0 ? &top[c - s] : nullptr, c - 2 * s >= 0);
+}
+
 template <class T, int K, bool SOLVE, bool SELINV, class Sink>
 ASVGP_HD void chain_phase3(const ChunkLayout& lay, int p, const ChainWork<T, K>& w, T* x_out, Sink& sink) {
     const int n_steps = lay.max_size();
diff --git a/asvgp_b200/csrc/banded_1d.cu b/asvgp_b200/csrc/banded_1d.cu
--- a/asvgp_b200/csrc/banded_1d.cu
+++ b/asvgp_b200/csrc/banded_1d.cu
@@ -104,66 +104,54 @@
 template <class T> struct ChainSpec { BandMat<T> A; VecRhs<T> rhs; };
 
 constexpr int kTraceBlocks = 64, kTraceThreads = 256, kTraceUnroll = 4;
-struct TraceJob {
-    const double* kstate;
-    const double* G;
-    double* tr_part;
-    int M, K, first_block;
-};
 __device__ __forceinline__ void trace_partial(const double* __restrict__ kstate, const double* __restrict__ G, int M, int K, int block,
                                               double* __restrict__ tr_part) {
     __shared__ double s_tr[2][kTraceThreads / 32];
     const Dual<1>* kinv = reinterpret_cast<const Dual<1>*>(kstate + 16);
-    double tr = 0.0, dtr_dl = 0.0;
     const int band = (K + 1) * M, stride = kTraceThreads * kTraceBlocks;
-    for (int i0 = block * kTraceThreads + threadIdx.x; i0 < band; i0 += stride * kTraceUnroll) {
-        Dual<1> sv[kTraceUnroll];
-        double gv[kTraceUnroll];
+    for (int vt = threadIdx.x; vt < kTraceThreads; vt += blockDim.x) {
+        double tr = 0.0, dtr_dl = 0.0;
+        for (int i0 = block * kTraceThreads + vt; i0 < band; i0 += stride * kTraceUnroll) {
+            Dual<1> sv[kTraceUnroll];
+            double gv[kTraceUnroll];
 #pragma unroll
-        for (int u = 0; u < kTraceUnroll; ++u) {
-            const int i = i0 + u * stride;
-            const int d = i / M, col = i - d * M;
-            const bool ok = i < band && col + d < M;
-            sv[u] = kinv[ok ? i : 0];
-            gv[u] = ok ? (d == 0 ? 1.0 : 2.0) * G[i] : 0.0;
-        }
+            for (int u = 0; u < kTraceUnroll; ++u) {
+                const int i = i0 + u * stride;
+                const int d = i / M, col = i - d * M;
+                const bool ok = i < band && col + d < M;
+                sv[u] = kinv[ok ? i : 0];
+                gv[u] = ok ? (d == 0 ? 1.0 : 2.0) * G[i] : 0.0;
+            }
 #pragma unroll
-        for (int u = 0; u < kTraceUnroll; ++u) {
-            if (gv[u] != 0.0) { tr = fma(sv[u].v, gv[u], tr); dtr_dl = fma(sv[u].d[0], gv[u], dtr_dl); }
-        }
-    }
+            for (int u = 0; u < kTraceUnroll; ++u) {
+                if (gv[u] != 0.0) { tr = fma(sv[u].v, gv[u], tr); dtr_dl = fma(sv[u].d[0], gv[u], dtr_dl); }
+            }
+        }
 #pragma unroll
-    for (int o = 16; o > 0; o >>= 1) {
-        tr += __shfl_xor_sync(0xffffffffu, tr, o);
-        dtr_dl += __shfl_xor_sync(0xffffffffu, dtr_dl, o);
-    }
-    if ((threadIdx.x & 31) == 0) { s_tr[0][threadIdx.x >> 5] = tr; s_tr[1][threadIdx.x >> 5] = dtr_dl; }
+        for (int o = 16; o > 0; o >>= 1) {
+            tr += __shfl_xor_sync(0xffffffffu, tr, o);
+            dtr_dl += __shfl_xor_sync(0xffffffffu, dtr_dl, o);
+        }
+        if ((vt & 31) == 0) { s_tr[0][vt >> 5] = tr; s_tr[1][vt >> 5] = dtr_dl; }
+    }
     __syncthreads();
     if (threadIdx.x == 0) {
-        tr = 0.0; dtr_dl = 0.0;
+        double tr = 0.0, dtr_dl = 0.0;
         for (int i = 0; i < kTraceThreads / 32; ++i) { tr += s_tr[0][i]; dtr_dl += s_tr[1][i]; }
         tr_part[2 * block] = tr; tr_part[2 * block + 1] = dtr_dl;
     }
+    __syncthreads();
 }
 
 template <class T, int K, int NCHAINS>
-__global__ void __launch_bounds__(256) chain_rows_kernel(ChunkLayout lay, ChainSpec<T> s0, ChainSpec<T> s1, ChainSpec<T> s2, ChainSpec<T> s3,
-                                                         T* __restrict__ out, unsigned* __restrict__ zero_me = nullptr,
-                                                         TraceJob trace = TraceJob{nullptr, nullptr, nullptr, 0, 0, 0}) {
-    pdl_launch_dependents();
-    if (zero_me != nullptr && blockIdx.x == 0 && threadIdx.x == 0) *zero_me = 0u;
-    if (trace.kstate != nullptr && (int)blockIdx.x >= trace.first_block) {
-        trace_partial(trace.kstate, trace.G, trace.M, trace.K, (int)blockIdx.x - trace.first_block, trace.tr_part);
-        return;
-    }
+__global__ void __launch_bounds__(256) chain_rows_kernel(ChunkLayout lay, ChainSpec<T> s0, ChainSpec<T> s1, T* __restrict__ out) {
     const unsigned n_rho = chain_n_rho(lay, K), P = lay.P;
     const unsigned per_chain = (unsigned)chain_rows_count<T, K>(lay);
     const unsigned total = per_chain * NCHAINS;
-    const unsigned n_row_blocks = trace.kstate != nullptr ? (unsigned)trace.first_block : gridDim.x;
-    for (unsigned t = blockIdx.x * blockDim.x + threadIdx.x; t < total; t += n_row_blocks * blockDim.x) {
+    for (unsigned t = blockIdx.x * blockDim.x + threadIdx.x; t < total; t += gridDim.x * blockDim.x) {
         const unsigned chain = t / per_chain;
         const unsigned e = t - chain * per_chain;
-        const ChainSpec<T>& sp = chain == 0 ? s0 : (chain == 1 ? s1 : (chain == 2 ? s2 : s3));
+        const ChainSpec<T>& sp = chain == 0 ? s0 : s1;
         const unsigned q = e / P;
         const int p = (int)(e - q * P);
         const int g0 = P > 1 ? lay.start(p) : 0;
@@ -348,100 +336,64 @@
 #undef ASVGP_STAMP
 }
 
-template <int K>
-struct ElboArgs {
+constexpr int kTicketSlot = 15;
+
+__device__ __forceinline__ void write_record(double* out, double logdet, double dlogdet, double quad, double dquad, int info,
+                                             const long long* clk) {
+    out[0] = logdet; out[1] = dlogdet;
+    out[2] = quad;   out[3] = dquad;
+    out[6] = (double)info;
+    const long long t_end = clock64();
+    out[8] = (double)(clk[1] - clk[0]); out[9] = (double)(clk[2] - clk[1]);
+    out[10] = (double)(clk[3] - clk[2]); out[11] = (double)(t_end - clk[3]);
+}
+
+template <int K>
+struct KuuChainArgs {
     ChunkLayout lay;
-    int first_chain;
-    ColumnStore<Dual<1>, K, true> cols[2];
-    double* partial[2];
-    const Dual<1>* rows;
+    ChainSpec<Dual<1>> spec;
+    ColumnStore<Dual<1>, K, true> cols;
+    double* record;
     Dual<1>* kinv;
 };
 
 template <int K>
-__global__ void __launch_bounds__(kChainThreads) elbo_chains_kernel(ElboArgs<K> a) {
+__device__ __forceinline__ void kuu_record(const KuuChainArgs<K>& a, const ChainTotals<Dual<1>, K>& tot, const long long* clk) {
+    write_record(a.record, tot.logdet.v, tot.logdet.d[0], tot.quad.v, tot.quad.d[0], tot.info, clk);
+    *reinterpret_cast<unsigned*>(a.record + kTicketSlot) = 0u;
+}
+
+template <int K>
+__global__ void __launch_bounds__(kChainThreads) elbo_kuu_kernel(KuuChainArgs<K> a) {
     using T = Dual<1>;
     extern __shared__ __align__(16) char smem[];
-    const int slot = blockIdx.x, chain = a.first_chain + slot, p = threadIdx.x;
-    const ChunkLayout lay = a.lay;
-    const int M = lay.M;
-    __shared__ ChainTotals<T, K> tot;
-    __shared__ long long clk[4];
-    double* out = a.partial[slot];
-    pdl_launch_dependents();
-    pdl_wait();
-
-    const int n_rho = chain_n_rho(lay, K), g0 = lay.P > 1 ? lay.start(p < lay.P ? p : 0) : 0, pp = p < lay.P ? p : 0;
-    const T* tab = a.rows + (size_t)slot * chain_rows_count<T, K>(lay);
-    const RowsMat<T, K> A{tab, g0, lay.P, pp, n_rho};
-    const RowsRhs<T> rhs{tab + (size_t)n_rho * (K + 1) * lay.P, g0, lay.P, pp, n_rho};
-    if (chain == 0) {
-        BandSink<T> sink{a.kinv, M};
-        run_chain<T, K, true, false, true>(lay, a.cols[slot], smem, A, rhs, static_cast<T*>(nullptr), sink, &tot, clk);
-    } else {
-        BandSink<T> no_sink{nullptr, M};
-        run_chain<T, K, false, false, false>(lay, a.cols[slot], smem, A, rhs, static_cast<T*>(nullptr), no_sink, &tot, clk);
-    }
-    if (p == 0) {
-        out[0] = tot.logdet.v; out[1] = tot.logdet.d[0];
-        out[2] = tot.quad.v;   out[3] = tot.quad.d[0];
-        out[6] = (double)tot.info;
-        const long long t_end = clock64();
-        out[8] = (double)(clk[1] - clk[0]); out[9] = (double)(clk[2] - clk[1]);
-        out[10] = (double)(clk[3] - clk[2]); out[11] = (double)(t_end - clk[3]);
-    }
-}
-
-template <int K, int NCTA>
-__global__ void __cluster_dims__(NCTA, 1, 1) __launch_bounds__(kChainThreads) elbo_chains_cluster_kernel(ElboArgs<K> a, Dual<1>* red_scratch) {
-    using T = Dual<1>;
-    extern __shared__ __align__(16) char smem[];
-    const int slot = blockIdx.x / NCTA, chain = a.first_chain + slot, rank = blockIdx.x % NCTA, tid = threadIdx.x;
+    const int p = threadIdx.x;
     const ChunkLayout lay = a.lay;
     __shared__ ChainTotals<T, K> tot;
     __shared__ long long clk[4];
-    double* out = a.partial[slot];
-    pdl_launch_dependents();
-    pdl_wait();
-    const int n_rho = chain_n_rho(lay, K);
-    const T* tab = a.rows + (size_t)slot * chain_rows_count<T, K>(lay);
-    T* scratch = red_scratch + (size_t)slot * ((size_t)(2 * K + 1) * lay.n_reduced() + 8);
-    auto g0_of = [&](int lane) { return lay.P > 1 ? lay.start(lane) : 0; };
-    auto make_A = [&](int lane) { return RowsMat<T, K>{tab, g0_of(lane), lay.P, lane, n_rho}; };
-    auto make_rhs = [&](int lane) { return RowsRhs<T>{tab + (size_t)n_rho * (K + 1) * lay.P, g0_of(lane), lay.P, lane, n_rho}; };
-    if (chain == 0) {
-        auto make_sink = [&](int) { return BandSink<T>{a.kinv, lay.M}; };
-        run_chain_cluster<T, K, true, false, true>(lay, a.cols[slot], smem, scratch, make_A, make_rhs, make_sink, static_cast<T*>(nullptr), &tot, clk);
-    } else {
-        auto make_sink = [&](int) { return BandSink<T>{nullptr, lay.M}; };
-        run_chain_cluster<T, K, false, false, false>(lay, a.cols[slot], smem, scratch, make_A, make_rhs, make_sink, static_cast<T*>(nullptr), &tot, clk);
-    }
-    if (rank == 0 && tid == 0) {
-        out[0] = tot.logdet.v; out[1] = tot.logdet.d[0];
-        out[2] = tot.quad.v;   out[3] = tot.quad.d[0];
-        out[6] = (double)tot.info;
-        const long long t_end = clock64();
-        out[8] = (double)(clk[1] - clk[0]); out[9] = (double)(clk[2] - clk[1]);
-        out[10] = (double)(clk[3] - clk[2]); out[11] = (double)(t_end - clk[3]);
-    }
-}
-
-__global__ void __launch_bounds__(kTraceThreads) elbo_finalize_kernel(const double* __restrict__ kstate, double* __restrict__ partial,
-                                                                      const double* __restrict__ G, const double* __restrict__ scal,
-                                                                      int M, int K, double variance, double sigma2, int trace_done,
-                                                                      double* __restrict__ out) {
-    double* tr_part = partial + 64;
-    unsigned* counter = reinterpret_cast<unsigned*>(partial + 32);
-    pdl_wait();
-    if (!trace_done) {
-        trace_partial(kstate, G, M, K, (int)blockIdx.x, tr_part);
-        if (threadIdx.x != 0) return;
-        __threadfence();
-        if (atomicAdd(counter, 1u) != gridDim.x - 1) return;
-        __threadfence();
-    } else if (threadIdx.x != 0) {
-        return;
-    }
+    BandSink<T> sink{a.kinv, lay.M};
+    run_chain<T, K, true, false, true>(lay, a.cols, smem, a.spec.A, a.spec.rhs, static_cast<T*>(nullptr), sink, &tot, clk);
+    if (p == 0) kuu_record(a, tot, clk);
+}
+
+template <int K, int NCTA>
+__global__ void __cluster_dims__(NCTA, 1, 1) __launch_bounds__(kChainThreads) elbo_kuu_cluster_kernel(KuuChainArgs<K> a, Dual<1>* red_scratch) {
+    using T = Dual<1>;
+    extern __shared__ __align__(16) char smem[];
+    const int rank = blockIdx.x % NCTA, tid = threadIdx.x;
+    const ChunkLayout lay = a.lay;
+    __shared__ ChainTotals<T, K> tot;
+    __shared__ long long clk[4];
+    auto make_A = [&](int) { return a.spec.A; };
+    auto make_rhs = [&](int) { return a.spec.rhs; };
+    auto make_sink = [&](int) { return BandSink<T>{a.kinv, lay.M}; };
+    run_chain_cluster<T, K, true, false, true>(lay, a.cols, smem, red_scratch, make_A, make_rhs, make_sink, static_cast<T*>(nullptr), &tot, clk);
+    if (rank == 0 && tid == 0) kuu_record(a, tot, clk);
+}
+
+__device__ void elbo_bound(const double* __restrict__ kstate, const double* partial, const double* __restrict__ scal, int M,
+                           double variance, double sigma2, double* __restrict__ out) {
+    const double* tr_part = partial + 64;
     double tr = 0.0, dtr_dl = 0.0;
     for (int i = 0; i < kTraceBlocks; ++i) { tr += __ldcg(tr_part + 2 * i); dtr_dl += __ldcg(tr_part + 2 * i + 1); }
     const double* cK = kstate;
@@ -450,8 +402,8 @@
     const double yy = scal[0], N = scal[1];
     const double v = variance, s2 = sigma2;
     const double logdetK = cK[0], dlogdetK_dl = cK[1];
-    const double logdetP = cL[0], dlogdetP_dl = cL[1], Q = cL[2], dQ_dl = cL[3];
-    const double dlogdetP_ds = cS[1], dQ_ds = cS[3];
+    const double logdetP = __ldcg(cL), dlogdetP_dl = __ldcg(cL + 1), Q = __ldcg(cL + 2), dQ_dl = __ldcg(cL + 3);
+    const double dlogdetP_ds = __ldcg(cS + 1), dQ_ds = __ldcg(cS + 3);
     const double two_pi = 6.283185307179586476925286766559;
     const double elbo = -0.5 * N * log(two_pi * s2) - 0.5 * logdetP + 0.5 * logdetK - 0.5 * yy / s2
                         + 0.5 * Q / (s2 * s2) - 0.5 * N * v / s2 + 0.5 * tr / s2;
@@ -465,12 +417,181 @@
     out[0] = elbo; out[1] = d_v; out[2] = d_l; out[3] = d_s;
     out[4] = logdetK; out[5] = logdetP; out[6] = Q; out[7] = tr;
     double info = cK[6];
-    if (info == 0.0) info = cL[6];
-    if (info == 0.0) info = cS[6];
+    if (info == 0.0) info = __ldcg(cL + 6);
+    if (info == 0.0) info = __ldcg(cS + 6);
     out[8] = info;
     out[9] = cK[8]; out[10] = cK[9]; out[11] = cK[10]; out[12] = cK[11];
-    out[13] = cL[8]; out[14] = cL[9];
+    out[13] = __ldcg(cL + 8); out[14] = __ldcg(cL + 9);
     out[15] = dtr_dl;
+}
+
+template <int K>
+struct PChainArgs {
+    ChunkLayout lay;
+    ChainSpec<Dual<1>> spec[2];
+    double* partial;
+    const double* kstate; const double* G; const double* scal;
+    double variance, sigma2;
+    double* out;
+    int n_arrivals;
+};
+
+template <int K>
+__device__ __forceinline__ void arrive(const PChainArgs<K>& a) {
+    unsigned* ticket = reinterpret_cast<unsigned*>(const_cast<double*>(a.kstate) + kTicketSlot);
+    __threadfence();
+    if (atomicAdd(ticket, 1u) != (unsigned)a.n_arrivals - 1u) return;
+    __threadfence();
+    *ticket = 0u;
+    elbo_bound(a.kstate, a.partial, a.scal, a.lay.M, a.variance, a.sigma2, a.out);
+}
+
+template <int K>
+__device__ __forceinline__ void pchain_record(const PChainArgs<K>& a, int chain, const ChainTotals<Dual<1>, K>& tot, const long long* clk) {
+    write_record(a.partial + 16 * chain, tot.logdet.v, tot.logdet.d[0], tot.quad.v, tot.quad.d[0], tot.info, clk);
+    if (a.kstate != nullptr) arrive(a);
+}
+
+template <int K>
+__device__ __forceinline__ void trace_ctas(const PChainArgs<K>& a, int i, int n) {
+    for (int v = i * (kTraceBlocks / n); v < (i + 1) * (kTraceBlocks / n); ++v) trace_partial(a.kstate, a.G, a.lay.M, K, v, a.partial + 64);
+    if (threadIdx.x == 0) arrive(a);
+}
+
+constexpr int kSingleTraceCTAs = 8;
+template <int K>
+__global__ void __launch_bounds__(kChainThreads) elbo_pchains_kernel(PChainArgs<K> a) {
+    using T = Dual<1>;
+    extern __shared__ __align__(16) char smem[];
+    const int chain = blockIdx.x, p = threadIdx.x;
+    const ChunkLayout lay = a.lay;
+    pdl_launch_dependents();
+    if (chain >= 2) { trace_ctas(a, chain - 2, kSingleTraceCTAs); return; }
+    if (a.kstate == nullptr && chain == 0 && p == 0) *reinterpret_cast<unsigned*>(a.partial + 32) = 0u;
+    __shared__ ChainTotals<T, K> tot;
+    __shared__ long long clk[4];
+    BandSink<T> no_sink{nullptr, lay.M};
+    const ColumnStore<T, K, true> no_store{nullptr, 0, 0};
+    run_chain<T, K, false, false, false>(lay, no_store, smem, a.spec[chain].A, a.spec[chain].rhs, static_cast<T*>(nullptr), no_sink, &tot, clk);
+    if (p == 0) pchain_record(a, chain, tot, clk);
+}
+
+template <int K, int NCTA>
+__global__ void __cluster_dims__(NCTA, 1, 1) __launch_bounds__(kChainThreads) elbo_pchains_cluster_kernel(PChainArgs<K> a) {
+    using T = Dual<1>;
+    namespace cg = cooperative_groups;
+    extern __shared__ __align__(16) char smem[];
+    constexpr int gs = kChainThreads;
+    const int chain = blockIdx.x / NCTA, rank = blockIdx.x % NCTA, tid = threadIdx.x;
+    const ChunkLayout lay = a.lay;
+    pdl_launch_dependents();
+    if (chain >= 2) { trace_ctas(a, rank, NCTA); return; }
+    if (a.kstate == nullptr && blockIdx.x == 0 && tid == 0) *reinterpret_cast<unsigned*>(a.partial + 32) = 0u;
+    cg::cluster_group cluster = cg::this_cluster();
+    __shared__ long long clk[4];
+    __shared__ CrNode<T, K> top[NCTA - 1];
+    __shared__ double s_tot[kChainThreads / 32][4];
+    __shared__ unsigned s_info[kChainThreads / 32];
+    __shared__ double s_cta[5];
+    ChainWork<T, K> w;
+    ChainSmall<T, K>::carve(gs + 2, smem, w);
+    ChunkSchur<T, K>* sch = w.schur;
+    CrNode<T, K>* loc = w.nodes;
+    const int p = rank * gs + tid, n = lay.P - 1;
+    const CrGroup g{n, gs, rank};
+
+    if (tid == 0) clk[0] = clock64();
+    {
+        const ColumnStore<T, K, true> no_store{nullptr, 0, 0};
+        eliminate_columns<T, K, true, false>(lay.start(p), lay.size(p), lay.max_size(), a.spec[chain].A, a.spec[chain].rhs, no_store, p, sch[tid]);
+    }
+    __syncthreads();
+    if (tid == 0) clk[1] = clock64();
+    const int j = tid + 1, ju = tid == 0 ? 0 : j;
+    if (j <= g.hi()) crg_assemble<T, K>(g, j, sch, loc);
+    if (tid == 0 && g.lo() == 0) crg_assemble<T, K>(g, 0, sch, loc);
+    __syncthreads();
+    for (int s = 1; s < gs; s *= 2) {
+        if (g.eliminates(s, j)) crg_eliminate<T, K>(g, s, j, lay.M, loc);
+        __syncthreads();
+        if (g.updates(s, ju)) crg_update<T, K>(g, s, ju, loc);
+        __syncthreads();
+    }
+    {
+        const ChunkSchur<T, K>& c = sch[tid];
+        T ld = c.logdet, qd = c.quad;
+        int info = c.info;
+        if (j < gs && j <= g.hi()) { ld += loc[j].logdet; qd += loc[j].quad; if (info == 0) info = loc[j].info; }
+        double v[4] = {value_of(ld), tangent_of(ld, 0), value_of(qd), tangent_of(qd, 0)};
+        unsigned uinfo = info == 0 ? 0xffffffffu : (unsigned)info;
+#pragma unroll
+        for (int o = 16; o > 0; o >>= 1) {
+#pragma unroll
+            for (int i = 0; i < 4; ++i) v[i] += __shfl_xor_sync(0xffffffffu, v[i], o);
+            uinfo = min(uinfo, __shfl_xor_sync(0xffffffffu, uinfo, o));
+        }
+        if ((tid & 31) == 0) { for (int i = 0; i < 4; ++i) s_tot[tid >> 5][i] = v[i]; s_info[tid >> 5] = uinfo; }
+        __syncthreads();
+        if (tid == 0) {
+            double t4[4] = {0, 0, 0, 0};
+            unsigned ui = 0xffffffffu;
+            for (int wv = 0; wv < kChainThreads / 32; ++wv) { for (int i = 0; i < 4; ++i) t4[i] += s_tot[wv][i]; ui = min(ui, s_info[wv]); }
+            for (int i = 0; i < 4; ++i) s_cta[i] = t4[i];
+            s_cta[4] = (double)ui;
+        }
+    }
+    cluster.sync();
+    if (rank == 0 && tid < 32) {
+        constexpr int nt = NCTA - 1;
+        if (tid < nt) crg_top_assemble<T, K>(tid, *cluster_peer(&loc[gs], tid), *cluster_peer(&loc[0], tid + 1), top[tid]);
+        __syncwarp();
+        for (int s = 1;; s *= 2) {
+            const int se = s < nt ? s : 0;
+            if (se > 0 ? tid < nt && (tid & (2 * s - 1)) == s : tid == 0) crg_top_eliminate<T, K>(nt, se, tid, gs, lay.M, top);
+            __syncwarp();
+            if (se == 0) break;
+            if (tid < nt && (tid & (2 * s - 1)) == 0) crg_top_update<T, K>(nt, s, tid, top);
+            __syncwarp();
+        }
+        if (tid == 0) {
+            double t4[4] = {0, 0, 0, 0};
+            double ui = 4294967295.0;
+            for (int r = 0; r < NCTA; ++r) {
+                const double* q = cluster_peer(s_cta, r);
+                for (int i = 0; i < 4; ++i) t4[i] += q[i];
+                ui = q[4] < ui ? q[4] : ui;
+            }
+            int info = ui >= 4294967295.0 ? 0 : (int)ui;
+            for (int t = 0; t < nt; ++t) {
+                t4[0] += value_of(top[t].logdet); t4[1] += tangent_of(top[t].logdet, 0);
+                t4[2] += value_of(top[t].quad);   t4[3] += tangent_of(top[t].quad, 0);
+                if (info == 0) info = top[t].info;
+            }
+            clk[2] = clock64();
+            s_cta[0] = t4[0]; s_cta[1] = t4[1]; s_cta[2] = t4[2]; s_cta[3] = t4[3];
+            s_info[0] = (unsigned)info;
+        }
+    }
+    cluster.sync();
+    if (rank == 0 && tid == 0) {
+        clk[3] = clock64();
+        write_record(a.partial + 16 * chain, s_cta[0], s_cta[1], s_cta[2], s_cta[3], (int)s_info[0], clk);
+        if (a.kstate != nullptr) arrive(a);
+    }
+}
+
+__global__ void __launch_bounds__(kTraceThreads) elbo_finalize_kernel(const double* __restrict__ kstate, double* __restrict__ partial,
+                                                                      const double* __restrict__ G, const double* __restrict__ scal,
+                                                                      int M, int K, double variance, double sigma2,
+                                                                      double* __restrict__ out) {
+    unsigned* counter = reinterpret_cast<unsigned*>(partial + 32);
+    pdl_wait();
+    trace_partial(kstate, G, M, K, (int)blockIdx.x, partial + 64);
+    if (threadIdx.x != 0) return;
+    __threadfence();
+    if (atomicAdd(counter, 1u) != gridDim.x - 1) return;
+    __threadfence();
+    elbo_bound(kstate, partial, scal, M, variance, sigma2, out);
 }
 
 template <int K>
@@ -566,7 +687,7 @@
         using T = Dual<1>;
         ChainSpec<T> s0{BandMat<T>{A, dA, nullptr, 0.0, 0.0, 1, lay.M}, VecRhs<T>{A, lay.M, 0}};
         const size_t total = chain_rows_count<T, K>(lay);
-        chain_rows_kernel<T, K, 1><<<(int)((total + 255) / 256), 256, 0, st>>>(lay, s0, s0, s0, s0, rows); ASVGP_LAUNCHED();
+        chain_rows_kernel<T, K, 1><<<(int)((total + 255) / 256), 256, 0, st>>>(lay, s0, s0, rows); ASVGP_LAUNCHED();
         ASVGP_CUDA_OK(cudaGetLastError());
     }
     ASVGP_CUDA_OK(cudaMemsetAsync(a.sig, 0, (size_t)(K + 1) * lay.M * sizeof(Dual<1>), st));
@@ -602,8 +723,7 @@
 static size_t red_scratch_count(const ChunkLayout& lay) { return (size_t)(2 * K + 1) * lay.n_reduced() + 8; }
 template <int K>
 static size_t chains_work_bytes(const ChunkLayout& lay, int n_chains) {
-    return n_chains * ChainPlan<Dual<1>, K>::bytes(lay) + kPartialBytes + align256(n_chains * chain_rows_count<Dual<1>, K>(lay) * sizeof(Dual<1>))
-           + align256(n_chains * red_scratch_count<K>(lay) * sizeof(Dual<1>));
+    return n_chains * ChainPlan<Dual<1>, K>::bytes(lay) + kPartialBytes + align256(n_chains * red_scratch_count<K>(lay) * sizeof(Dual<1>));
 }
 static size_t kuu_state_doubles(int M, int K) { return 16 + 2 * (size_t)(K + 1) * M; }
 template <int K>
@@ -616,66 +736,8 @@
            + 256 + (((size_t)lay.M * sizeof(double) + 255) & ~(size_t)255) + 2 * chain_rows_count<double, K>(lay) * sizeof(double) + 256;
 }
 
-template <int K>
-static int launch_chain_group(const ChunkLayout& lay, int first_chain, int n_chains, const ChainSpec<Dual<1>>& s0,
-                              const ChainSpec<Dual<1>>& s1, double* partial0, Dual<1>* kinv, char* work, double** partials_out,
-                              cudaEvent_t gate, TraceJob trace, cudaStream_t st) {
-    using T = Dual<1>;
-    ElboArgs<K> a;
-    a.lay = lay;
-    a.first_chain = first_chain;
-    a.kinv = kinv;
-    char* p = work;
-    for (int c = 0; c < 2; ++c) {
-        a.cols[c] = ChainPlan<T, K>::carve(lay, c < n_chains ? p : work);
-        if (c < n_chains) p += ChainPlan<T, K>::bytes(lay);
-    }
-    double* partial = reinterpret_cast<double*>(p);
-    p += kPartialBytes;
-    a.partial[0] = partial0 != nullptr ? partial0 : partial;
-    a.partial[1] = partial + 16;
-    if (partials_out != nullptr) *partials_out = partial;
-    T* rows = reinterpret_cast<T*>(p);
-    p += align256(n_chains * chain_rows_count<T, K>(lay) * sizeof(T));
-    a.rows = rows;
-    T* scratch = reinterpret_cast<T*>(p);
-    const size_t total = n_chains * chain_rows_count<T, K>(lay);
-    ASVGP_REQUIRE(total < ((size_t)1 << 31), "banded chains: %zu row-table entries exceed the 32-bit index range", total);
-    const int grid = (int)std::min<size_t>((total + 255) / 256, 148 * 8);
-    if (n_chains == 1) {
-        chain_rows_kernel<T, K, 1><<<grid, 256, 0, st>>>(lay, s0, s0, s0, s0, rows);
-    } else {
-        trace.first_block = grid;
-        trace.tr_part = partial + 64;
-        chain_rows_kernel<T, K, 2><<<grid + (trace.kstate != nullptr ? kTraceBlocks : 0), 256, 0, st>>>(
-            lay, s0, s1, s1, s1, rows, reinterpret_cast<unsigned*>(partial + 32), trace);
-    }
-    ASVGP_LAUNCHED();
-    ASVGP_CUDA_OK(cudaGetLastError());
-    if (gate != nullptr) ASVGP_CUDA_OK(cudaEventRecord(gate, st));
-    const int n_cta = (lay.P + kChainThreads - 1) / kChainThreads;
-    const bool pdl = gate == nullptr;
-    const size_t smem_floor = gate != nullptr ? (size_t)(227 * 1024 - 2048) : 0;
-    if (n_cta > 1) {
-        const size_t smem = std::max(ChainSmall<T, K>::bytes(kChainThreads + 1), smem_floor);
-        if (n_cta == 2) {
-            ASVGP_CUDA_OK(allow_smem(elbo_chains_cluster_kernel<K, 2>, smem));
-            ASVGP_CUDA_OK(launch_dependent(elbo_chains_cluster_kernel<K, 2>, n_chains * 2, kChainThreads, smem, st, pdl, a, scratch));
-        } else if (n_cta == 8) {
-            ASVGP_CUDA_OK(allow_smem(elbo_chains_cluster_kernel<K, 8>, smem));
-            ASVGP_CUDA_OK(launch_dependent(elbo_chains_cluster_kernel<K, 8>, n_chains * 8, kChainThreads, smem, st, pdl, a, scratch));
-        } else {
-            ASVGP_CUDA_OK(allow_smem(elbo_chains_cluster_kernel<K, 4>, smem));
-            ASVGP_CUDA_OK(launch_dependent(elbo_chains_cluster_kernel<K, 4>, n_chains * 4, kChainThreads, smem, st, pdl, a, scratch));
-        }
-    } else {
-        const size_t smem = std::max(ChainSmall<T, K>::bytes(lay.P), smem_floor);
-        ASVGP_CUDA_OK(allow_smem(elbo_chains_kernel<K>, smem));
-        ASVGP_CUDA_OK(launch_dependent(elbo_chains_kernel<K>, n_chains, kChainThreads, smem, st, pdl, a));
-    }
-    ASVGP_LAUNCHED();
-    ASVGP_CUDA_OK(cudaGetLastError());
-    return kOk;
+static size_t chain_smem(size_t need, bool beside_streaming) {
+    return std::max(need, beside_streaming ? (size_t)(227 * 1024 - 2048) : (size_t)0);
 }
 
 template <int K>
@@ -683,9 +745,37 @@
                             cudaStream_t st) {
     using T = Dual<1>;
     const int M = lay.M;
-    ChainSpec<T> s0{BandMat<T>{Kuu, dKuu, nullptr, 0.0, 0.0, 1, M}, VecRhs<T>{Kuu, M, 0}};
-    return launch_chain_group<K>(lay, 0, 1, s0, s0, kstate, reinterpret_cast<T*>(kstate + 16), work, nullptr, gate,
-                                 TraceJob{nullptr, nullptr, nullptr, 0, 0, 0}, st);
+    KuuChainArgs<K> a;
+    a.lay = lay;
+    a.spec = ChainSpec<T>{BandMat<T>{Kuu, dKuu, nullptr, 0.0, 0.0, 1, M}, VecRhs<T>{Kuu, M, 0}};
+    a.record = kstate;
+    a.kinv = reinterpret_cast<T*>(kstate + 16);
+    char* p = work;
+    a.cols = ChainPlan<T, K>::carve(lay, p);
+    p += ChainPlan<T, K>::bytes(lay) + kPartialBytes;
+    T* scratch = reinterpret_cast<T*>(p);
+    if (gate != nullptr) ASVGP_CUDA_OK(cudaEventRecord(gate, st));
+    const int n_cta = (lay.P + kChainThreads - 1) / kChainThreads;
+    if (n_cta > 1) {
+        const size_t smem = chain_smem(ChainSmall<T, K>::bytes(kChainThreads + 1), gate != nullptr);
+        if (n_cta == 2) {
+            ASVGP_CUDA_OK(allow_smem(elbo_kuu_cluster_kernel<K, 2>, smem));
+            elbo_kuu_cluster_kernel<K, 2><<<2, kChainThreads, smem, st>>>(a, scratch);
+        } else if (n_cta == 8) {
+            ASVGP_CUDA_OK(allow_smem(elbo_kuu_cluster_kernel<K, 8>, smem));
+            elbo_kuu_cluster_kernel<K, 8><<<8, kChainThreads, smem, st>>>(a, scratch);
+        } else {
+            ASVGP_CUDA_OK(allow_smem(elbo_kuu_cluster_kernel<K, 4>, smem));
+            elbo_kuu_cluster_kernel<K, 4><<<4, kChainThreads, smem, st>>>(a, scratch);
+        }
+    } else {
+        const size_t smem = chain_smem(ChainSmall<T, K>::bytes(lay.P), gate != nullptr);
+        ASVGP_CUDA_OK(allow_smem(elbo_kuu_kernel<K>, smem));
+        elbo_kuu_kernel<K><<<1, kChainThreads, smem, st>>>(a);
+    }
+    ASVGP_LAUNCHED();
+    ASVGP_CUDA_OK(cudaGetLastError());
+    return kOk;
 }
 
 template <int K>
@@ -696,16 +786,48 @@
     const double* G = acc;
     const double* b = acc + (size_t)(K + 1) * M;
     const double inv_s2 = 1.0 / sigma2;
-    ChainSpec<T> s1{BandMat<T>{Kuu, dKuu, G, inv_s2, 0.0, 1, M}, VecRhs<T>{b, M, 1}};
-    ChainSpec<T> s2{BandMat<T>{Kuu, dKuu, G, inv_s2, -inv_s2 * inv_s2, 0, M}, VecRhs<T>{b, M, 1}};
-    double* partial = nullptr;
-    if (!join_late && kuu_ready != nullptr) ASVGP_CUDA_OK(cudaStreamWaitEvent(st, kuu_ready, 0));
-    const TraceJob trace{join_late ? nullptr : kstate, G, nullptr, M, K, 0};
-    if (int rc = launch_chain_group<K>(lay, 1, 2, s1, s2, nullptr, nullptr, work, &partial, nullptr, trace, st)) return rc;
-    if (join_late && kuu_ready != nullptr) ASVGP_CUDA_OK(cudaStreamWaitEvent(st, kuu_ready, 0));
-    const bool pdl = !(join_late && kuu_ready != nullptr);
-    ASVGP_CUDA_OK(launch_dependent(elbo_finalize_kernel, join_late ? kTraceBlocks : 1, kTraceThreads, 0, st, pdl, kstate, partial, G,
-                                   acc + (size_t)(K + 2) * M, M, K, variance, sigma2, join_late ? 0 : 1, out));
+    PChainArgs<K> a;
+    a.lay = lay;
+    a.spec[0] = ChainSpec<T>{BandMat<T>{Kuu, dKuu, G, inv_s2, 0.0, 1, M}, VecRhs<T>{b, M, 1}};
+    a.spec[1] = ChainSpec<T>{BandMat<T>{Kuu, dKuu, G, inv_s2, -inv_s2 * inv_s2, 0, M}, VecRhs<T>{b, M, 1}};
+    char* p = work + 2 * ChainPlan<T, K>::bytes(lay);
+    a.partial = reinterpret_cast<double*>(p);
+    const bool fused = !join_late;
+    a.kstate = fused ? kstate : nullptr;
+    a.G = G;
+    a.scal = acc + (size_t)(K + 2) * M;
+    a.variance = variance; a.sigma2 = sigma2;
+    a.out = out;
+    if (fused && kuu_ready != nullptr) ASVGP_CUDA_OK(cudaStreamWaitEvent(st, kuu_ready, 0));
+    const int n_cta = (lay.P + kChainThreads - 1) / kChainThreads;
+    if (n_cta > 1) {
+        ASVGP_REQUIRE(lay.P == n_cta * kChainThreads, "banded chains: %d chunks do not fill %d CTAs", lay.P, n_cta);
+        a.n_arrivals = 2 + n_cta;
+        const int grid = (fused ? 3 : 2) * n_cta;
+        const size_t smem = ChainSmall<T, K>::bytes(kChainThreads + 2);
+        if (n_cta == 2) {
+            ASVGP_CUDA_OK(allow_smem(elbo_pchains_cluster_kernel<K, 2>, smem));
+            elbo_pchains_cluster_kernel<K, 2><<<grid, kChainThreads, smem, st>>>(a);
+        } else if (n_cta == 8) {
+            ASVGP_CUDA_OK(allow_smem(elbo_pchains_cluster_kernel<K, 8>, smem));
+            elbo_pchains_cluster_kernel<K, 8><<<grid, kChainThreads, smem, st>>>(a);
+        } else {
+            ASVGP_CUDA_OK(allow_smem(elbo_pchains_cluster_kernel<K, 4>, smem));
+            elbo_pchains_cluster_kernel<K, 4><<<grid, kChainThreads, smem, st>>>(a);
+        }
+    } else {
+        a.n_arrivals = 2 + kSingleTraceCTAs;
+        const size_t smem = ChainSmall<T, K>::bytes(lay.P);
+        ASVGP_CUDA_OK(allow_smem(elbo_pchains_kernel<K>, smem));
+        elbo_pchains_kernel<K><<<2 + (fused ? kSingleTraceCTAs : 0), kChainThreads, smem, st>>>(a);
+    }
+    ASVGP_LAUNCHED();
+    ASVGP_CUDA_OK(cudaGetLastError());
+    if (fused) return kOk;
+    if (kuu_ready != nullptr) ASVGP_CUDA_OK(cudaStreamWaitEvent(st, kuu_ready, 0));
+    const bool pdl = kuu_ready == nullptr;
+    ASVGP_CUDA_OK(launch_dependent(elbo_finalize_kernel, kTraceBlocks, kTraceThreads, 0, st, pdl, kstate, a.partial, G, a.scal, M, K,
+                                   variance, sigma2, out));
     ASVGP_LAUNCHED();
     ASVGP_CUDA_OK(cudaGetLastError());
     return kOk;
@@ -743,7 +865,7 @@
         ChainSpec<T> s0{BandMat<T>{Kuu, nullptr, nullptr, 0.0, 0.0, 0, M}, VecRhs<T>{Kuu, M, 0}};
         ChainSpec<T> s1{BandMat<T>{Kuu, nullptr, a.G, 1.0 / sigma2, 0.0, 0, M}, VecRhs<T>{a.b, M, 1}};
         const size_t total = 2 * chain_rows_count<T, K>(lay);
-        chain_rows_kernel<T, K, 2><<<(int)std::min<size_t>((total + 255) / 256, 148 * 8), 256, 0, st>>>(lay, s0, s1, s1, s1, rows); ASVGP_LAUNCHED();
+        chain_rows_kernel<T, K, 2><<<(int)std::min<size_t>((total + 255) / 256, 148 * 8), 256, 0, st>>>(lay, s0, s1, rows); ASVGP_LAUNCHED();
         ASVGP_CUDA_OK(cudaGetLastError());
     }
     ASVGP_CUDA_OK(cudaMemsetAsync(a.sigK, 0, 2 * band_bytes, st));
```

After: 300.0 billion (median of 6 runs). 1.03x the previous value.
